# PengNi/deepsignal-plant

Hardware: NVIDIA B200
Metric: classified sites/sec (ModelBiLSTM both_bilstm bn13_sn16 hidden 256) (higher is better)
Workload: dtype f16 operands / f32 accumulate

## Files before the change

deepsignal_plant_b200/csrc/kernels_tc.cu:

```cuda
#include "tc.cuh"
#include "tc_prims.cuh"
#include <vector>
#include <cstring>
#include <cstdlib>

namespace dsp {

using namespace tc;

namespace {

constexpr int TILE = 128;
constexpr int SLAB_BYTES = TILE * SLAB_ROW_BYTES;
constexpr int HSLAB_BYTES = SLAB_BYTES / 2;
constexpr int EPI_WARPS = 16;
constexpr int NTHREADS = 128 + EPI_WARPS * 32;
constexpr int CPT = 128 / (EPI_WARPS / 4);
constexpr int UPT = CPT / 4;
constexpr float LOG2E = 1.4426950408889634f;
constexpr uint16_t PAIR_MASK = 3;

#ifndef DSP_POLY_MASK
#define DSP_POLY_MASK 0
#endif
#ifndef DSP_POLY_MASK_BRANCH
#define DSP_POLY_MASK_BRANCH 3
#endif
#ifndef DSP_POLY_MASK_L0
#define DSP_POLY_MASK_L0 DSP_POLY_MASK
#endif
#ifndef DSP_PW32_ALL
#define DSP_PW32_ALL 0
#endif
#ifndef DSP_DIR_INTERLEAVE
#define DSP_DIR_INTERLEAVE 1
#endif
#ifndef DSP_MERGE_RCP
#define DSP_MERGE_RCP 1
#endif
#ifndef DSP_TANH_APPROX
#define DSP_TANH_APPROX 2
#endif

struct LayerParams {
    const uint8_t* x_img;
    const uint8_t* w_img;
    const float* bias;
    const float* h0;
    const float* c0;
    uint64_t seed;
    uint32_t rng_call;
    uint32_t rng_slot;
    int64_t site_base;
    int64_t state_dir_stride;
    uint8_t* y_img;
    float* hfinal;
    int64_t n;
    int T;
    int xk16;
    int y_slabs;
    int y_col_off;
    int write_y;
    const float* w2t;
    const float* b2;
    float* logits;
    float* probs;
    int32_t* labels;
    int num_classes;
};

enum { MODE_LSTM = 0, MODE_FC = 1, MODE_HEAD = 2 };
constexpr int HEAD_MAX_CLASSES = 8;
template <int KSX, int MODE> struct RingCfg {
    static constexpr int STG = KSX >= 8 ? 2 : 4;
    static constexpr int NST = KSX >= 8 ? (MODE == 2 ? 4 : 5) : (MODE == 1 ? 2 : 4);
    static constexpr int XB = (MODE == 1 && KSX <= 4) ? 2 : 1;
};

__device__ __forceinline__ float4 philox_normal4(uint32_t c0, uint32_t c1, uint32_t c2, uint32_t c3, uint32_t k0, uint32_t k1) {
#pragma unroll
    for (int r = 0; r < 10; ++r) {
        const uint32_t hi0 = __umulhi(0xD2511F53u, c0), lo0 = 0xD2511F53u * c0;
        const uint32_t hi1 = __umulhi(0xCD9E8D57u, c2), lo1 = 0xCD9E8D57u * c2;
        c0 = hi1 ^ c1 ^ k0; c1 = lo1; c2 = hi0 ^ c3 ^ k1; c3 = lo0;
        k0 += 0x9E3779B9u; k1 += 0xBB67AE85u;
    }
    const float u0 = ((float)c0 + 1.0f) * 2.3283064365386963e-10f, u1 = (float)c1 * 2.3283064365386963e-10f;
    const float u2 = ((float)c2 + 1.0f) * 2.3283064365386963e-10f, u3 = (float)c3 * 2.3283064365386963e-10f;
    const float r0 = sqrtf(-2.0f * __logf(u0)), r1 = sqrtf(-2.0f * __logf(u2));
    float s0, cs0, s1, cs1;
    __sincosf(6.283185307179586f * u1, &s0, &cs0);
    __sincosf(6.283185307179586f * u3, &s1, &cs1);
    return make_float4(r0 * cs0, r0 * s0, r1 * cs1, r1 * s1);
}

template <bool POLY, bool HI_CLAMP>
__device__ __forceinline__ float2 exp2_pair(float2 x) {
    if constexpr (POLY) {
        x.x = fmaxf(fminf(x.x, 40.f), -126.f);
        x.y = fmaxf(fminf(x.y, 40.f), -126.f);
        const float MG = 12582912.f;
        const float2 t = add2(x, make_float2(MG, MG));
        const float2 r = add2(t, make_float2(-MG, -MG));
        const float2 f = fma2(r, make_float2(-1.f, -1.f), x);
        float2 q = fma2(make_float2(0.0013390863f, 0.0013390863f), f, make_float2(0.009676032f, 0.009676032f));
        q = fma2(q, f, make_float2(0.05550357f, 0.05550357f));
        q = fma2(q, f, make_float2(0.24022107f, 0.24022107f));
        q = fma2(q, f, make_float2(0.6931472f, 0.6931472f));
        q = fma2(q, f, make_float2(1.0000001f, 1.0000001f));
        q.x = __int_as_float(__float_as_int(q.x) + (__float_as_int(t.x) << 23));
        q.y = __int_as_float(__float_as_int(q.y) + (__float_as_int(t.y) << 23));
        return q;
    } else {
        if constexpr (HI_CLAMP) { x.x = fminf(x.x, 40.f); x.y = fminf(x.y, 40.f); }
        return make_float2(ex2_approx(x.x), ex2_approx(x.y));
    }
}

__device__ __forceinline__ float tanh_approx(float x) {
    float y;
    asm("tanh.approx.f32 %0, %1;" : "=f"(y) : "f"(x));
    return y;
}
__host__ __device__ inline float gate_scale(int g) {
#if DSP_TANH_APPROX == 2
    return g == 2 ? 1.f : 0.5f;
#elif DSP_TANH_APPROX == 1
    return g == 2 ? -2.f * 1.4426950408889634f : (g == 3 ? 0.5f : -1.4426950408889634f);
#else
    return g == 2 ? -2.f * 1.4426950408889634f : -1.4426950408889634f;
#endif
}

template <int PM>
__device__ __forceinline__ void lstm_cell2(float2 ai, float2 af, float2 ag, float2 ao, float2& c, float2& h) {
    const float2 ONE = make_float2(1.f, 1.f), NEG1 = make_float2(-1.f, -1.f);
#ifdef DSP_EPI_STUB
    c = fma2(af, make_float2(1e-3f, 1e-3f), c);
    h = fma2(add2(ai, add2(ag, ao)), make_float2(1e-2f, 1e-2f), mul2(c, make_float2(1e-3f, 1e-3f)));
    return;
#endif
#if DSP_TANH_APPROX == 2
    {
        const float2 HALF = make_float2(0.5f, 0.5f);
        const float2 si = fma2(make_float2(tanh_approx(ai.x), tanh_approx(ai.y)), HALF, HALF);
        const float2 sf = fma2(make_float2(tanh_approx(af.x), tanh_approx(af.y)), HALF, HALF);
        const float2 so = fma2(make_float2(tanh_approx(ao.x), tanh_approx(ao.y)), HALF, HALF);
        const float2 tg = make_float2(tanh_approx(ag.x), tanh_approx(ag.y));
        c = fma2(sf, c, mul2(si, tg));
        h = mul2(so, make_float2(tanh_approx(c.x), tanh_approx(c.y)));
        return;
    }
#endif
#if DSP_MERGE_RCP
    constexpr bool CLAMP_IF = true;
#else
    constexpr bool CLAMP_IF = false;
#endif
    const float2 ei = exp2_pair<((PM >> 2) & 1) != 0, CLAMP_IF>(ai);
    const float2 ef = exp2_pair<((PM >> 3) & 1) != 0, CLAMP_IF>(af);
    const float2 eg = exp2_pair<(PM & 1) != 0, true>(ag);
    const float2 eo = exp2_pair<((PM >> 4) & 1) != 0, false>(ao);
#if DSP_MERGE_RCP
    const float2 F = add2(ef, ONE);
    const float2 AG = mul2(add2(ei, ONE), add2(eg, ONE));
    const float2 num = fma2(c, AG, mul2(fma2(eg, NEG1, ONE), F));
    const float2 den = mul2(F, AG);
    const float2 cn = mul2(num, make_float2(rcp_approx(den.x), rcp_approx(den.y)));
#else
    const float2 F = add2(ef, ONE);
    const float2 sf = make_float2(rcp_approx(F.x), rcp_approx(F.y));
    const float2 AG = mul2(add2(ei, ONE), add2(eg, ONE));
    const float2 rg = make_float2(rcp_approx(AG.x), rcp_approx(AG.y));
    const float2 ig = mul2(fma2(eg, NEG1, ONE), rg);
    const float2 cn = fma2(sf, c, ig);
#endif
    c = cn;
#if DSP_TANH_APPROX == 1
    {
        const float2 HALF = make_float2(0.5f, 0.5f);
        const float2 so = fma2(make_float2(tanh_approx(ao.x), tanh_approx(ao.y)), HALF, HALF);
        h = mul2(so, make_float2(tanh_approx(cn.x), tanh_approx(cn.y)));
        return;
    }
#endif
    const float2 ec = exp2_pair<((PM >> 1) & 1) != 0, true>(mul2(cn, make_float2(-2.f * LOG2E, -2.f * LOG2E)));
    const float2 D = mul2(add2(eo, ONE), add2(ec, ONE));
    const float2 rd = make_float2(rcp_approx(D.x), rcp_approx(D.y));
    h = mul2(fma2(ec, NEG1, ONE), rd);
}

template <int KSX, int H, int MODE, int NOUT>
__global__ void __launch_bounds__(NTHREADS, 1)
layer_kernel(const LayerParams p) {
    constexpr bool IS_FC = MODE != MODE_LSTM;
    constexpr int STG = RingCfg<KSX, MODE>::STG, NST = RingCfg<KSX, MODE>::NST, XB = RingCfg<KSX, MODE>::XB;
    constexpr int NXS = KSX * XB;
    constexpr int NCH = IS_FC ? NOUT / 128 : H / 32;
    constexpr int KSH = IS_FC ? 0 : H / 64;
    constexpr int KS = KSX + KSH;
    constexpr int W_STEP = NCH * KS;
    constexpr int NBIAS = NCH * 128;
    constexpr uint32_t IDESC = make_idesc_f16(256, 128);
    static_assert(W_STEP % STG == 0, "a step must be a whole number of ring stages");
    static_assert(IS_FC || NCH % 2 == 0, "chunks are issued in pairs");
    static_assert(EPI_WARPS == 16 && CPT == 32 && UPT == 8, "the epilogue code below is written for 32-column slices");

    extern __shared__ __align__(1024) uint8_t smem_raw[];
    uint8_t* smem = (uint8_t*)(((uintptr_t)smem_raw + 1023) & ~(uintptr_t)1023);
    uint8_t* s_x = smem;
    uint8_t* s_w = smem + (size_t)NXS * SLAB_BYTES;
    float* s_bias = reinterpret_cast<float*>(s_w + (size_t)NST * STG * HSLAB_BYTES);
    __shared__ __align__(8) uint64_t bars[2 * NST + 2 * NXS + 5];
    __shared__ uint32_t tmem_base_s;
    const uint32_t b_wfull = smem_u32(&bars[0]), b_wempty = smem_u32(&bars[NST]);
    const uint32_t b_xfull = smem_u32(&bars[2 * NST]), b_xempty = smem_u32(&bars[2 * NST + NXS]);
    const uint32_t b_accfull = smem_u32(&bars[2 * NST + 2 * NXS]), b_accempty = b_accfull + 16;
    const uint32_t b_hready = b_accfull + 32;

    const int tid = threadIdx.x, warp = tid >> 5, lane = tid & 31;
#if DSP_DIR_INTERLEAVE
    const int dir = IS_FC ? 0 : (int)((blockIdx.x >> 1) & 1u);
    const int tile = IS_FC ? (int)blockIdx.x : (int)(((blockIdx.x >> 2) << 1) | (blockIdx.x & 1u));
#else
    const int tile = blockIdx.x, dir = IS_FC ? 0 : blockIdx.y;
#endif
    const int T = p.T;
    const uint32_t crank = cluster_ctarank();

    if (tid == 0) {
        const uint32_t both = crank == 0 ? 2u : 1u;
        for (int i = 0; i < NST; ++i) { mbar_init(b_wfull + 8 * i, both); mbar_init(b_wempty + 8 * i, 1); }
        for (int i = 0; i < NXS; ++i) { mbar_init(b_xfull + 8 * i, both); mbar_init(b_xempty + 8 * i, 1); }
        for (int i = 0; i < 2; ++i) { mbar_init(b_accfull + 8 * i, 1); mbar_init(b_accempty + 8 * i, 2 * EPI_WARPS); }
        mbar_init(b_hready, 2 * EPI_WARPS);
        mbar_fence_init();
    }
    if (warp == 3) tmem_alloc_pair(smem_u32(&tmem_base_s), 512);
    tc_fence_before();
    __syncthreads();
    cluster_sync_all();
    tc_fence_after();
    const uint32_t tmem = tmem_base_s;
    griddep_launch_dependents();
    const uint32_t t_acc = tmem;
    const uint32_t t_h = tmem + 256;

    if (warp < 4) {
        asm volatile("setmaxnreg.dec.sync.aligned.u32 32;");
        if (warp == 0) {
            if (elect_one()) {
                const size_t total = (size_t)(MODE == MODE_HEAD ? T : 1) * W_STEP;
                const uint8_t* wsrc = p.w_img + ((size_t)dir * 2 + crank) * total * HSLAB_BYTES;
                uint32_t stage = 0, phase = 0;
                for (int step = 0; step < T; ++step) {
                    const uint8_t* src = wsrc + (size_t)(MODE == MODE_HEAD ? step : 0) * W_STEP * HSLAB_BYTES;
                    for (int s = 0; s < W_STEP; s += STG) {
                        mbar_wait(b_wempty + 8 * stage, phase ^ 1);
                        mbar_arrive_expect_tx(b_wfull + 8 * stage, STG * HSLAB_BYTES);
                        bulk_g2s(smem_u32(s_w + (size_t)stage * STG * HSLAB_BYTES), src, STG * HSLAB_BYTES, b_wfull + 8 * stage);
                        src += (size_t)STG * HSLAB_BYTES;
                        if (++stage == NST) { stage = 0; phase ^= 1; }
                    }
                }
            }
        } else if (warp == 2) {
            if (elect_one()) {
                griddep_wait();
                for (int step = 0; step < T; ++step) {
                    const int t = dir ? (T - 1 - step) : step;
                    const uint8_t* xsrc = (MODE == MODE_HEAD)
                        ? p.x_img + ((size_t)tile * 2 + (step == 1 ? 1 : 0)) * KSX * SLAB_BYTES
                        : p.x_img + ((size_t)tile * T + t) * KSX * SLAB_BYTES;
                    const int xbuf = step % XB, xround = step / XB;
                    for (int j = 0; j < KSX; ++j) {
                        const int xi = xbuf * KSX + j;
                        mbar_wait(b_xempty + 8 * xi, (xround & 1) ^ 1);
                        mbar_arrive_expect_tx(b_xfull + 8 * xi, SLAB_BYTES);
                        bulk_g2s(smem_u32(s_x + (size_t)xi * SLAB_BYTES), xsrc + (size_t)j * SLAB_BYTES, SLAB_BYTES, b_xfull + 8 * xi);
                    }
                }
            }
        } else if (warp == 1 && crank != 0) {
            const uint32_t r_wfull = mapa_u32(b_wfull, 0), r_xfull = mapa_u32(b_xfull, 0);
            uint32_t stage = 0, phase = 0;
            for (int step = 0; step < T; ++step) {
                for (int j = 0; j < KSX; ++j) {
                    const int xi = (step % XB) * KSX + j;
                    mbar_wait(b_xfull + 8 * xi, (step / XB) & 1);
                    if (lane == 0) mbar_arrive_cluster(r_xfull + 8 * xi);
                }
                for (int s = 0; s < W_STEP; s += STG) {
                    mbar_wait(b_wfull + 8 * stage, phase);
                    if (lane == 0) mbar_arrive_cluster(r_wfull + 8 * stage);
                    if (++stage == NST) { stage = 0; phase ^= 1; }
                }
            }
        } else if (warp == 1) {
            const bool leader = elect_one();
            const uint32_t a_lo0 = smem_desc_lo(smem_u32(s_x)), b_lo0 = smem_desc_lo(smem_u32(s_w));
            const int xk16 = p.xk16;
            uint32_t stage = 0, phase = 0, in_stage = 0;
            auto w_acquire = [&]() -> uint32_t {
                if (in_stage == 0) { mbar_wait_cluster(b_wfull + 8 * stage, phase); tc_fence_after(); }
                return b_lo0 + (stage * STG + in_stage) * (uint32_t)(HSLAB_BYTES >> 4);
            };
            auto w_release = [&]() {
                if (++in_stage == STG) {
                    if (leader) mma2_commit(b_wempty + 8 * stage, PAIR_MASK);
                    in_stage = 0;
                    if (++stage == NST) { stage = 0; phase ^= 1; }
                }
                __syncwarp();
            };
            auto issue_x = [&](uint32_t acc, bool fresh, bool first_use, bool last_use, int step) {
#pragma unroll
                for (int j = 0; j < KSX; ++j) {
                    const int xi = (step % XB) * KSX + j;
                    if (first_use) { mbar_wait_cluster(b_xfull + 8 * xi, (step / XB) & 1); tc_fence_after(); }
                    const uint32_t bl = w_acquire();
                    if (leader) {
                        const uint32_t al = a_lo0 + (uint32_t)xi * (SLAB_BYTES >> 4);
                        const int nk = (KSX * 4 == xk16) ? 4 : min(4, xk16 - 4 * j);
#pragma unroll
                        for (int k = 0; k < 4; ++k) {
                            if (k < nk) {
                                if (j == 0 && k == 0 && fresh) mma2_ss_lo<0>(acc, al, bl, IDESC);
                                else mma2_ss_lo<1>(acc, al + k * 2, bl + k * 2, IDESC);
                            }
                        }
                        if (last_use) mma2_commit(b_xempty + 8 * xi, PAIR_MASK);
                    }
                    w_release();
                }
            };
            for (int step = 0; step < T; ++step) {
                if constexpr (MODE == MODE_LSTM) {
                    const uint32_t a_t = t_h + (uint32_t)(step & 1) * 128u;
                    for (int pr = 0; pr < NCH / 2; ++pr) {
                        const uint32_t use = (uint32_t)(step * (NCH / 2) + pr);
#pragma unroll
                        for (int e = 0; e < 2; ++e) {
                            mbar_wait_cluster(b_accempty + 8 * e, (use & 1u) ^ 1u);
                            tc_fence_after();
                            issue_x(t_acc + e * 128u, true, pr == 0 && e == 0, pr == NCH / 2 - 1 && e == 1, step);
                        }
                        if (pr == 0) { mbar_wait_cluster(b_hready, step & 1); tc_fence_after(); }
#pragma unroll
                        for (int e = 0; e < 2; ++e) {
#pragma unroll
                            for (int j = 0; j < KSH; ++j) {
                                const uint32_t bl = w_acquire();
                                if (leader) {
#pragma unroll
                                    for (int k = 0; k < 4; ++k)
                                        mma2_ts_lo<1>(t_acc + e * 128u, a_t + (uint32_t)(j * 32 + k * 8), bl + k * 2, IDESC);
                                }
                                w_release();
                            }
                            if (leader) mma2_commit(b_accfull + 8 * e, PAIR_MASK);
                            __syncwarp();
                        }
                    }
                } else {
                    for (int ch = 0; ch < NCH; ++ch) {
                        const uint32_t g = (MODE == MODE_HEAD) ? (uint32_t)ch : (uint32_t)(step * NCH + ch);
                        const uint32_t buf = g & 1u, use = g >> 1;
                        const bool fresh = (MODE != MODE_HEAD) || step == 0;
                        if (MODE != MODE_HEAD) { mbar_wait_cluster(b_accempty + 8 * buf, (use & 1u) ^ 1u); tc_fence_after(); }
                        issue_x(t_acc + buf * 128u, fresh, ch == 0, ch == NCH - 1, step);
                        if (leader && (MODE != MODE_HEAD || step == T - 1)) mma2_commit(b_accfull + 8 * buf, PAIR_MASK);
                        __syncwarp();
                    }
                }
            }
        }
    } else {
        asm volatile("setmaxnreg.inc.sync.aligned.u32 112;");
        const int ew = warp - 4;
        const int q = warp & 3;
        const int sl = ew >> 2;
        const int row = q * 32 + lane;
        const int64_t site = (int64_t)tile * TILE + row;
        const bool valid = site < p.n;
        const uint32_t lane_addr = (uint32_t)(q * 32) << 16;
        const uint32_t r_accempty = mapa_u32(b_accempty, 0), r_hready = mapa_u32(b_hready, 0);

        for (int i = tid - 128; i < NBIAS; i += EPI_WARPS * 32) s_bias[i] = p.bias[(size_t)dir * NBIAS + i];
        asm volatile("bar.sync 1, %0;" ::"n"(EPI_WARPS * 32) : "memory");

        if constexpr (MODE == MODE_HEAD) {
            __shared__ float head_part[EPI_WARPS / 4][TILE][HEAD_MAX_CLASSES];
            const int C = p.num_classes;
            float part_sum[HEAD_MAX_CLASSES];
#pragma unroll
            for (int cc = 0; cc < HEAD_MAX_CLASSES; ++cc) part_sum[cc] = 0.f;
#pragma unroll
            for (int ch = 0; ch < NCH; ++ch) {
                const uint32_t buf = (uint32_t)ch & 1u, use = (uint32_t)ch >> 1;
                mbar_wait(b_accfull + 8 * buf, use & 1u);
                tc_fence_after();
                uint32_t v[32];
                tmem_ld32(t_acc + buf * 128u + lane_addr + (uint32_t)(sl * CPT), v);
                tmem_ld_wait();
#pragma unroll
                for (int j = 0; j < 32; ++j) {
                    const int col = ch * 128 + sl * CPT + j;
                    const float z = fmaxf(__uint_as_float(v[j]) + s_bias[col], 0.f);
#pragma unroll
                    for (int cc = 0; cc < HEAD_MAX_CLASSES; ++cc)
                        if (cc < C) part_sum[cc] = fmaf(z, __ldg(p.w2t + (size_t)col * C + cc), part_sum[cc]);
                }
            }
#pragma unroll
            for (int cc = 0; cc < HEAD_MAX_CLASSES; ++cc) head_part[sl][row][cc] = part_sum[cc];
            asm volatile("bar.sync 1, %0;" ::"n"(EPI_WARPS * 32) : "memory");
            if (sl == 0 && valid) {
                float lg[HEAD_MAX_CLASSES];
                float mx = -3.0e38f;
                int arg = 0;
#pragma unroll
                for (int cc = 0; cc < HEAD_MAX_CLASSES; ++cc) {
                    lg[cc] = 0.f;
                    if (cc < C) {
                        float a = __ldg(p.b2 + cc);
#pragma unroll
                        for (int s4 = 0; s4 < EPI_WARPS / 4; ++s4) a += head_part[s4][row][cc];
                        lg[cc] = a;
                        if (lg[cc] > mx) { mx = lg[cc]; arg = cc; }
                    }
                }
                float sum = 0.f;
#pragma unroll
                for (int cc = 0; cc < HEAD_MAX_CLASSES; ++cc) if (cc < C) sum += expf(lg[cc] - mx);
#pragma unroll
                for (int cc = 0; cc < HEAD_MAX_CLASSES; ++cc)
                    if (cc < C) {
                        p.logits[site * C + cc] = lg[cc];
                        p.probs[site * C + cc] = expf(lg[cc] - mx) / sum;
                    }
                if (p.labels) p.labels[site] = arg;
            }
        } else if constexpr (MODE == MODE_FC) {
            for (int step = 0; step < T; ++step) {
                uint8_t* ybase = p.y_img + ((size_t)tile * T + step) * p.y_slabs * SLAB_BYTES;
#pragma unroll
                for (int ch = 0; ch < NCH; ++ch) {
                    const uint32_t g = (uint32_t)(step * NCH + ch);
                    const uint32_t buf = g & 1u, use = g >> 1;
                    mbar_wait(b_accfull + 8 * buf, use & 1u);
                    tc_fence_after();
                    const int col0 = p.y_col_off + ch * 128 + sl * CPT;
                    uint8_t* yslab = ybase + (size_t)(col0 >> 6) * SLAB_BYTES + row * SLAB_ROW_BYTES;
                    uint32_t v[32];
                    tmem_ld32(t_acc + buf * 128u + lane_addr + (uint32_t)(sl * CPT), v);
                    tmem_ld_wait();
                    tc_fence_before();
                    __syncwarp();
                    if (lane == 0) mbar_arrive_cluster(r_accempty + 8 * buf);
                    const float* bs = s_bias + ch * 128 + sl * CPT;
#pragma unroll
                    for (int c8 = 0; c8 < 4; ++c8) {
                        uint32_t o[4];
#pragma unroll
                        for (int e = 0; e < 4; ++e) {
                            const int j = c8 * 8 + e * 2;
                            const float a = fmaxf(__uint_as_float(v[j]) + bs[j], 0.f);
                            const float b = fmaxf(__uint_as_float(v[j + 1]) + bs[j + 1], 0.f);
                            o[e] = pack_half2(a, b);
                        }
                        const int chunk = ((col0 & 63) >> 3) + c8;
                        *reinterpret_cast<uint4*>(yslab + ((chunk ^ (row & 7)) << 4)) = make_uint4(o[0], o[1], o[2], o[3]);
                    }
                }
            }
        } else {
            float2 c2[NCH][UPT / 2];
            const bool draw = p.h0 == nullptr;
            const uint64_t gs = (uint64_t)(p.site_base + site);
            const uint32_t k0 = (uint32_t)p.seed, k1 = (uint32_t)(p.seed >> 32);
            const uint32_t slot0 = (p.rng_slot + (uint32_t)dir) << 16;
            if (draw) {
#pragma unroll 1
                for (int i = 0; i < NCH * (UPT / 4); ++i) {
                    const int unit = (i / (UPT / 4)) * 32 + sl * UPT + (i % (UPT / 4)) * 4;
                    const float4 hq = philox_normal4((uint32_t)gs, (uint32_t)(gs >> 32), slot0 | (uint32_t)(unit >> 2), p.rng_call, k0, k1);
                    tmem_st2(t_h + lane_addr + (uint32_t)(unit >> 1), pack_half2(hq.x, hq.y), pack_half2(hq.z, hq.w));
                }
                tmem_st_wait();
            } else {
                const float* h0 = p.h0 + (size_t)dir * p.state_dir_stride + (size_t)site * H;
                const float* c0 = p.c0 + (size_t)dir * p.state_dir_stride + (size_t)site * H;
#pragma unroll
                for (int ch = 0; ch < NCH; ++ch) {
                    const int u0 = ch * 32 + sl * UPT;
                    float4 cv0 = make_float4(0.f, 0.f, 0.f, 0.f), cv1 = cv0, hq0 = cv0, hq1 = cv0;
                    if (valid) {
                        cv0 = *reinterpret_cast<const float4*>(c0 + u0); cv1 = *reinterpret_cast<const float4*>(c0 + u0 + 4);
                        hq0 = *reinterpret_cast<const float4*>(h0 + u0); hq1 = *reinterpret_cast<const float4*>(h0 + u0 + 4);
                    }
                    c2[ch][0] = make_float2(cv0.x, cv0.y); c2[ch][1] = make_float2(cv0.z, cv0.w);
                    c2[ch][2] = make_float2(cv1.x, cv1.y); c2[ch][3] = make_float2(cv1.z, cv1.w);
                    tmem_st4(t_h + lane_addr + (uint32_t)(u0 >> 1), pack_half2(hq0.x, hq0.y), pack_half2(hq0.z, hq0.w),
                             pack_half2(hq1.x, hq1.y), pack_half2(hq1.z, hq1.w));
                }
                tmem_st_wait();
            }
            tc_fence_before();
            __syncwarp();
            if (lane == 0) mbar_arrive_cluster(r_hready);
            if (draw) {
                const uint32_t t_park = t_h + 128u + lane_addr;
#pragma unroll 1
                for (int i = 0; i < NCH * (UPT / 4); ++i) {
                    const int unit = (i / (UPT / 4)) * 32 + sl * UPT + (i % (UPT / 4)) * 4;
                    const float4 cv = philox_normal4((uint32_t)gs, (uint32_t)(gs >> 32), slot0 | (uint32_t)(unit >> 2) | 0x8000u, p.rng_call, k0, k1);
                    tmem_st2(t_park + (uint32_t)(unit >> 1), pack_half2(cv.x, cv.y), pack_half2(cv.z, cv.w));
                }
                tmem_st_wait();
#pragma unroll
                for (int ch = 0; ch < NCH; ++ch) {
                    uint32_t v[4];
                    tmem_ld4(t_park + (uint32_t)((ch * 32 + sl * UPT) >> 1), v);
                    tmem_ld_wait();
#pragma unroll
                    for (int j = 0; j < UPT / 2; ++j) {
                        const __half2 hh = *reinterpret_cast<const __half2*>(&v[j]);
                        c2[ch][j] = make_float2(__low2float(hh), __high2float(hh));
                    }
                }
            }
            const uint32_t s_bias_u32 = smem_u32(s_bias) + (uint32_t)(sl * CPT * 4);
            for (int step = 0; step < T; ++step) {
                const int t = dir ? (T - 1 - step) : step;
                const bool last = (step == T - 1);
                uint8_t* ybase = p.y_img + ((size_t)tile * (p.write_y == 2 ? 2 : T) + (p.write_y == 2 ? 0 : t)) * p.y_slabs * SLAB_BYTES
                                 + row * SLAB_ROW_BYTES;
                const bool do_write = p.write_y == 1 || (p.write_y == 2 && last);
                const uint32_t t_hnext = t_h + (uint32_t)((step + 1) & 1) * 128u + lane_addr;
#pragma unroll
                for (int ch = 0; ch < NCH; ++ch) {
                    const uint32_t buf = (uint32_t)ch & 1u;
                    const uint32_t use = (uint32_t)(step * (NCH / 2) + (ch >> 1));
                    mbar_wait(b_accfull + 8 * buf, use & 1u);
                    tc_fence_after();
                    const int u0 = ch * 32 + sl * UPT;
                    float2 h2[UPT / 2];
                    constexpr int PW = (H == 128 || DSP_PW32_ALL) ? 32 : 16;
#pragma unroll
                    for (int part = 0; part < CPT / PW; ++part) {
                        uint32_t v[PW];
                        if constexpr (PW == 32) tmem_ld32(t_acc + buf * 128u + lane_addr + (uint32_t)(sl * CPT), reinterpret_cast<uint32_t(&)[32]>(v));
                        else tmem_ld16(t_acc + buf * 128u + lane_addr + (uint32_t)(sl * CPT + part * 16), reinterpret_cast<uint32_t(&)[16]>(v));
                        float4 bq[PW / 4];
#pragma unroll
                        for (int i = 0; i < PW / 4; ++i) bq[i] = lds128(s_bias_u32 + (uint32_t)((ch * 128 + part * PW + i * 4) * 4));
                        tmem_ld_wait();
                        if (part == CPT / PW - 1) {
                            tc_fence_before();
                            __syncwarp();
                            if (lane == 0) mbar_arrive_cluster(r_accempty + 8 * buf);
                        }
#pragma unroll
                        for (int qq = 0; qq < PW / 8; ++qq) {
                            const float4 b0 = bq[2 * qq], b1 = bq[2 * qq + 1];
                            const float2 ai = add2(make_float2(__uint_as_float(v[qq * 8 + 0]), __uint_as_float(v[qq * 8 + 1])), make_float2(b0.x, b0.y));
                            const float2 af = add2(make_float2(__uint_as_float(v[qq * 8 + 2]), __uint_as_float(v[qq * 8 + 3])), make_float2(b0.z, b0.w));
                            const float2 ag = add2(make_float2(__uint_as_float(v[qq * 8 + 4]), __uint_as_float(v[qq * 8 + 5])), make_float2(b1.x, b1.y));
                            const float2 ao = add2(make_float2(__uint_as_float(v[qq * 8 + 6]), __uint_as_float(v[qq * 8 + 7])), make_float2(b1.z, b1.w));
                            lstm_cell2<(H == 128) ? DSP_POLY_MASK_BRANCH : (KSX == 4 ? DSP_POLY_MASK_L0 : DSP_POLY_MASK)>(ai, af, ag, ao, c2[ch][part * (PW / 8) + qq], h2[part * (PW / 8) + qq]);
                        }
                    }
                    uint32_t pk[UPT / 2];
#pragma unroll
                    for (int j = 0; j < UPT / 2; ++j) pk[j] = pack_half2(h2[j].x, h2[j].y);
                    tmem_st4(t_hnext + (uint32_t)(u0 >> 1), pk[0], pk[1], pk[2], pk[3]);
                    if (do_write) {
                        const int col = dir * H + u0;
                        uint8_t* yslab = ybase + (size_t)(col >> 6) * SLAB_BYTES;
                        const int chunk = (col & 63) >> 3;
                        *reinterpret_cast<uint4*>(yslab + (((chunk) ^ (row & 7)) << 4)) = make_uint4(pk[0], pk[1], pk[2], pk[3]);
                        if (p.write_y == 2) {
                            uint32_t lo[UPT / 2];
#pragma unroll
                            for (int j = 0; j < UPT / 2; ++j) {
                                const __half2 hh = *reinterpret_cast<const __half2*>(&pk[j]);
                                lo[j] = pack_half2(h2[j].x - __low2float(hh), h2[j].y - __high2float(hh));
                            }
                            uint8_t* lslab = yslab + (size_t)p.y_slabs * SLAB_BYTES;
                            *reinterpret_cast<uint4*>(lslab + (((chunk) ^ (row & 7)) << 4)) = make_uint4(lo[0], lo[1], lo[2], lo[3]);
                        }
                    }
                    if (last && p.hfinal != nullptr && valid) {
                        float* hf = p.hfinal + (size_t)site * (2 * H) + dir * H + u0;
#pragma unroll
                        for (int j = 0; j < UPT / 2; j += 2)
                            *reinterpret_cast<float4*>(hf + 2 * j) = make_float4(h2[j].x, h2[j].y, h2[j + 1].x, h2[j + 1].y);
                    }
                }
                tmem_st_wait();
                tc_fence_before();
                __syncwarp();
                if (lane == 0) mbar_arrive_cluster(r_hready);
            }
        }
    }
    tc_fence_before();
    __syncthreads();
    cluster_sync_all();
    if (warp == 3) tmem_dealloc_pair(tmem, 512);
}

constexpr int BR_H = 128, BR_NW = 64, BR_NCH = BR_H / 16, BR_KSH = BR_H / 64;
constexpr int QSLAB_BYTES = 32 * SLAB_ROW_BYTES;
constexpr int BR_STG = 4, BR_NST = 6;

template <int KSX>
__global__ void __launch_bounds__(NTHREADS, 1)
branch_kernel(const LayerParams p) {
    constexpr int KS = KSX + BR_KSH;
    constexpr int PAIR_UNITS = 4 * KSX + 4 * BR_KSH;
    constexpr int W_STEP = (BR_NCH / 2) * PAIR_UNITS;
    constexpr int NBIAS = 2 * BR_NCH * BR_NW;
    constexpr uint32_t IDESC = make_idesc_f16(256, BR_NW);
    static_assert(W_STEP % BR_STG == 0 && KS * 2 == PAIR_UNITS / 2, "stream layout");

    extern __shared__ __align__(1024) uint8_t smem_raw[];
    uint8_t* smem = (uint8_t*)(((uintptr_t)smem_raw + 1023) & ~(uintptr_t)1023);
    uint8_t* s_x = smem;
    uint8_t* s_w = smem + (size_t)2 * KSX * SLAB_BYTES;
    float* s_bias = reinterpret_cast<float*>(s_w + (size_t)BR_NST * BR_STG * QSLAB_BYTES);
    __shared__ __align__(8) uint64_t bars[2 * BR_NST + 4 * KSX + 10];
    __shared__ uint32_t tmem_base_s;
    const uint32_t b_wfull = smem_u32(&bars[0]), b_wempty = smem_u32(&bars[BR_NST]);
    const uint32_t b_xfull = smem_u32(&bars[2 * BR_NST]), b_xempty = b_xfull + 8 * 2 * KSX;
    const uint32_t b_accfull = b_xempty + 8 * 2 * KSX, b_accempty = b_accfull + 32;
    const uint32_t b_hready = b_accempty + 32;

    const int tid = threadIdx.x, warp = tid >> 5, lane = tid & 31;
    const int tile = blockIdx.x;
    const int T = p.T;
    const uint32_t crank = cluster_ctarank();

    if (tid == 0) {
        const uint32_t both = crank == 0 ? 2u : 1u;
        for (int i = 0; i < BR_NST; ++i) { mbar_init(b_wfull + 8 * i, both); mbar_init(b_wempty + 8 * i, 1); }
        for (int i = 0; i < 2 * KSX; ++i) { mbar_init(b_xfull + 8 * i, both); mbar_init(b_xempty + 8 * i, 1); }
        for (int i = 0; i < 4; ++i) { mbar_init(b_accfull + 8 * i, 1); mbar_init(b_accempty + 8 * i, EPI_WARPS); }
        for (int i = 0; i < 2; ++i) mbar_init(b_hready + 8 * i, EPI_WARPS);
        mbar_fence_init();
    }
    if (warp == 3) tmem_alloc_pair(smem_u32(&tmem_base_s), 512);
    tc_fence_before();
    __syncthreads();
    cluster_sync_all();
    tc_fence_after();
    const uint32_t tmem = tmem_base_s;
    griddep_launch_dependents();
    auto t_acc = [&](int d, int e) -> uint32_t { return tmem + (uint32_t)(d * 128 + e * 64); };
    auto t_h = [&](int d, int b) -> uint32_t { return tmem + 256u + (uint32_t)(d * 128 + b * 64); };

    if (warp < 4) {
        asm volatile("setmaxnreg.dec.sync.aligned.u32 32;");
        if (warp == 0) {
            if (elect_one()) {
                const uint8_t* wsrc = p.w_img + (size_t)crank * W_STEP * QSLAB_BYTES;
                uint32_t stage = 0, phase = 0;
                for (int step = 0; step < T; ++step) {
                    const uint8_t* src = wsrc;
                    for (int s = 0; s < W_STEP; s += BR_STG) {
                        mbar_wait(b_wempty + 8 * stage, phase ^ 1);
                        mbar_arrive_expect_tx(b_wfull + 8 * stage, BR_STG * QSLAB_BYTES);
                        bulk_g2s(smem_u32(s_w + (size_t)stage * BR_STG * QSLAB_BYTES), src, BR_STG * QSLAB_BYTES, b_wfull + 8 * stage);
                        src += (size_t)BR_STG * QSLAB_BYTES;
                        if (++stage == BR_NST) { stage = 0; phase ^= 1; }
                    }
                }
            }
        } else if (warp == 2) {
            if (elect_one()) {
                griddep_wait();
                for (int step = 0; step < T; ++step)
                    for (int d = 0; d < 2; ++d) {
                        const int t = d ? (T - 1 - step) : step;
                        const uint8_t* xsrc = p.x_img + ((size_t)tile * T + t) * KSX * SLAB_BYTES;
                        for (int j = 0; j < KSX; ++j) {
                            const uint32_t o = 8u * (uint32_t)(d * KSX + j);
                            mbar_wait(b_xempty + o, (step & 1) ^ 1);
                            mbar_arrive_expect_tx(b_xfull + o, SLAB_BYTES);
                            bulk_g2s(smem_u32(s_x + (size_t)(d * KSX + j) * SLAB_BYTES), xsrc + (size_t)j * SLAB_BYTES, SLAB_BYTES, b_xfull + o);
                        }
                    }
            }
        } else if (warp == 1 && crank != 0) {
            const uint32_t r_wfull = mapa_u32(b_wfull, 0), r_xfull = mapa_u32(b_xfull, 0);
            uint32_t stage = 0, phase = 0;
            for (int step = 0; step < T; ++step) {
                for (int i = 0; i < 2 * KSX; ++i) {
                    mbar_wait(b_xfull + 8 * i, step & 1);
                    if (lane == 0) mbar_arrive_cluster(r_xfull + 8 * i);
                }
                for (int s = 0; s < W_STEP; s += BR_STG) {
                    mbar_wait(b_wfull + 8 * stage, phase);
                    if (lane == 0) mbar_arrive_cluster(r_wfull + 8 * stage);
                    if (++stage == BR_NST) { stage = 0; phase ^= 1; }
                }
            }
        } else if (warp == 1) {
            const bool leader = elect_one();
            const uint32_t a_lo0 = smem_desc_lo(smem_u32(s_x)), b_lo0 = smem_desc_lo(smem_u32(s_w));
            const int xk16 = p.xk16;
            uint32_t stage = 0, phase = 0, in_stage = 0;
            auto w_acquire = [&]() -> uint32_t {
                if (in_stage == 0) { mbar_wait_cluster(b_wfull + 8 * stage, phase); tc_fence_after(); }
                return b_lo0 + (stage * BR_STG + in_stage) * (uint32_t)(QSLAB_BYTES >> 4);
            };
            auto w_release = [&]() {
                if (++in_stage == BR_STG) {
                    if (leader) mma2_commit(b_wempty + 8 * stage, PAIR_MASK);
                    in_stage = 0;
                    if (++stage == BR_NST) { stage = 0; phase ^= 1; }
                }
                __syncwarp();
            };
            for (int step = 0; step < T; ++step) {
                for (int pr = 0; pr < BR_NCH / 2; ++pr) {
                    const uint32_t use = (uint32_t)(step * (BR_NCH / 2) + pr);
#pragma unroll
                    for (int d = 0; d < 2; ++d)
#pragma unroll
                        for (int e = 0; e < 2; ++e) {
                            mbar_wait_cluster(b_accempty + 8 * (d * 2 + e), (use & 1u) ^ 1u);
                            tc_fence_after();
#pragma unroll
                            for (int j = 0; j < KSX; ++j) {
                                const uint32_t xo = 8u * (uint32_t)(d * KSX + j);
                                if (pr == 0 && e == 0) { mbar_wait_cluster(b_xfull + xo, step & 1); tc_fence_after(); }
                                const uint32_t bl = w_acquire();
                                if (leader) {
                                    const uint32_t al = a_lo0 + (uint32_t)(d * KSX + j) * (SLAB_BYTES >> 4);
                                    const int nk = (KSX * 4 == xk16) ? 4 : min(4, xk16 - 4 * j);
#pragma unroll
                                    for (int k = 0; k < 4; ++k) {
                                        if (k < nk) {
                                            if (j == 0 && k == 0) mma2_ss_lo<0>(t_acc(d, e), al, bl, IDESC);
                                            else mma2_ss_lo<1>(t_acc(d, e), al + k * 2, bl + k * 2, IDESC);
                                        }
                                    }
                                    if (pr == BR_NCH / 2 - 1 && e == 1) mma2_commit(b_xempty + xo, PAIR_MASK);
                                }
                                w_release();
                            }
                        }
#pragma unroll
                    for (int d = 0; d < 2; ++d) {
                        if (pr == 0) { mbar_wait_cluster(b_hready + 8 * d, step & 1); tc_fence_after(); }
                        const uint32_t a_t = t_h(d, step & 1);
#pragma unroll
                        for (int e = 0; e < 2; ++e) {
#pragma unroll
                            for (int j = 0; j < BR_KSH; ++j) {
                                const uint32_t bl = w_acquire();
                                if (leader) {
#pragma unroll
                                    for (int k = 0; k < 4; ++k)
                                        mma2_ts_lo<1>(t_acc(d, e), a_t + (uint32_t)(j * 32 + k * 8), bl + k * 2, IDESC);
                                }
                                w_release();
                            }
                            if (leader) mma2_commit(b_accfull + 8 * (d * 2 + e), PAIR_MASK);
                            __syncwarp();
                        }
                    }
                }
            }
        }
    } else {
        asm volatile("setmaxnreg.inc.sync.aligned.u32 112;");
        const int ew = warp - 4;
        const int d = ew >> 3;
        const int q = warp & 3;
        const int half = (ew >> 2) & 1;
        const int row = q * 32 + lane;
        const int64_t site = (int64_t)tile * TILE + row;
        const bool valid = site < p.n;
        const uint32_t lane_addr = (uint32_t)(q * 32) << 16;
        const uint32_t r_accempty = mapa_u32(b_accempty, 0) + 16u * (uint32_t)d, r_hready = mapa_u32(b_hready, 0) + 8u * (uint32_t)d;
        const uint32_t b_myfull = b_accfull + 16u * (uint32_t)d;

        for (int i = tid - 128; i < NBIAS; i += EPI_WARPS * 32) s_bias[i] = p.bias[i];
        asm volatile("bar.sync 1, %0;" ::"n"(EPI_WARPS * 32) : "memory");

        constexpr int UPT = 8;
        float2 c2[BR_NCH][UPT / 2];
        const bool draw = p.h0 == nullptr;
        const uint64_t gs = (uint64_t)(p.site_base + site);
        const uint32_t k0 = (uint32_t)p.seed, k1 = (uint32_t)(p.seed >> 32);
        const uint32_t slot0 = (p.rng_slot + (uint32_t)d) << 16;
        if (draw) {
#pragma unroll 1
            for (int i = 0; i < BR_NCH * (UPT / 4); ++i) {
                const int unit = (i >> 1) * 16 + half * UPT + (i & 1) * 4;
                const float4 hq = philox_normal4((uint32_t)gs, (uint32_t)(gs >> 32), slot0 | (uint32_t)(unit >> 2), p.rng_call, k0, k1);
                tmem_st2(t_h(d, 0) + lane_addr + (uint32_t)(unit >> 1), pack_half2(hq.x, hq.y), pack_half2(hq.z, hq.w));
            }
            tmem_st_wait();
        } else {
            const float* h0 = p.h0 + (size_t)d * p.state_dir_stride + (size_t)site * BR_H;
            const float* c0 = p.c0 + (size_t)d * p.state_dir_stride + (size_t)site * BR_H;
#pragma unroll
            for (int ch = 0; ch < BR_NCH; ++ch) {
                const int u0 = ch * 16 + half * UPT;
                float4 cv0 = make_float4(0.f, 0.f, 0.f, 0.f), cv1 = cv0, hq0 = cv0, hq1 = cv0;
                if (valid) {
                    cv0 = *reinterpret_cast<const float4*>(c0 + u0); cv1 = *reinterpret_cast<const float4*>(c0 + u0 + 4);
                    hq0 = *reinterpret_cast<const float4*>(h0 + u0); hq1 = *reinterpret_cast<const float4*>(h0 + u0 + 4);
                }
                c2[ch][0] = make_float2(cv0.x, cv0.y); c2[ch][1] = make_float2(cv0.z, cv0.w);
                c2[ch][2] = make_float2(cv1.x, cv1.y); c2[ch][3] = make_float2(cv1.z, cv1.w);
                tmem_st4(t_h(d, 0) + lane_addr + (uint32_t)(u0 >> 1), pack_half2(hq0.x, hq0.y), pack_half2(hq0.z, hq0.w),
                         pack_half2(hq1.x, hq1.y), pack_half2(hq1.z, hq1.w));
            }
            tmem_st_wait();
        }
        tc_fence_before();
        __syncwarp();
        if (lane == 0) mbar_arrive_cluster(r_hready);
        if (draw) {
            const uint32_t t_park = t_h(d, 1) + lane_addr;
#pragma unroll 1
            for (int i = 0; i < BR_NCH * (UPT / 4); ++i) {
                const int unit = (i >> 1) * 16 + half * UPT + (i & 1) * 4;
                const float4 cv = philox_normal4((uint32_t)gs, (uint32_t)(gs >> 32), slot0 | (uint32_t)(unit >> 2) | 0x8000u, p.rng_call, k0, k1);
                tmem_st2(t_park + (uint32_t)(unit >> 1), pack_half2(cv.x, cv.y), pack_half2(cv.z, cv.w));
            }
            tmem_st_wait();
#pragma unroll
            for (int ch = 0; ch < BR_NCH; ++ch) {
                uint32_t v[4];
                tmem_ld4(t_park + (uint32_t)((ch * 16 + half * UPT) >> 1), v);
                tmem_ld_wait();
#pragma unroll
                for (int j = 0; j < UPT / 2; ++j) {
                    const __half2 hh = *reinterpret_cast<const __half2*>(&v[j]);
                    c2[ch][j] = make_float2(__low2float(hh), __high2float(hh));
                }
            }
        }
        const uint32_t s_bias_u32 = smem_u32(s_bias) + (uint32_t)((d * BR_NCH * BR_NW + half * 32) * 4);
        for (int step = 0; step < T; ++step) {
            const int t = d ? (T - 1 - step) : step;
            uint8_t* ybase = p.y_img + ((size_t)tile * T + t) * p.y_slabs * SLAB_BYTES + row * SLAB_ROW_BYTES;
            const uint32_t t_hnext = t_h(d, (step + 1) & 1) + lane_addr;
#pragma unroll
            for (int ch = 0; ch < BR_NCH; ++ch) {
                const int e = ch & 1;
                const uint32_t use = (uint32_t)(step * (BR_NCH / 2) + (ch >> 1));
                mbar_wait(b_myfull + 8 * e, use & 1u);
                tc_fence_after();
                const int u0 = ch * 16 + half * UPT;
                float2 h2[UPT / 2];
#pragma unroll
                for (int part = 0; part < 2; ++part) {
                    uint32_t v[16];
                    tmem_ld16(t_acc(d, e) + lane_addr + (uint32_t)(half * 32 + part * 16), v);
                    float4 bq[4];
#pragma unroll
                    for (int i = 0; i < 4; ++i) bq[i] = lds128(s_bias_u32 + (uint32_t)((ch * BR_NW + part * 16 + i * 4) * 4));
                    tmem_ld_wait();
                    if (part == 1) {
                        tc_fence_before();
                        __syncwarp();
                        if (lane == 0) mbar_arrive_cluster(r_accempty + 8 * e);
                    }
#pragma unroll
                    for (int qq = 0; qq < 2; ++qq) {
                        const float4 b0 = bq[2 * qq], b1 = bq[2 * qq + 1];
                        const float2 ai = add2(make_float2(__uint_as_float(v[qq * 8 + 0]), __uint_as_float(v[qq * 8 + 1])), make_float2(b0.x, b0.y));
                        const float2 af = add2(make_float2(__uint_as_float(v[qq * 8 + 2]), __uint_as_float(v[qq * 8 + 3])), make_float2(b0.z, b0.w));
                        const float2 ag = add2(make_float2(__uint_as_float(v[qq * 8 + 4]), __uint_as_float(v[qq * 8 + 5])), make_float2(b1.x, b1.y));
                        const float2 ao = add2(make_float2(__uint_as_float(v[qq * 8 + 6]), __uint_as_float(v[qq * 8 + 7])), make_float2(b1.z, b1.w));
                        lstm_cell2<DSP_POLY_MASK_BRANCH>(ai, af, ag, ao, c2[ch][part * 2 + qq], h2[part * 2 + qq]);
                    }
                }
                uint32_t pk[UPT / 2];
#pragma unroll
                for (int j = 0; j < UPT / 2; ++j) pk[j] = pack_half2(h2[j].x, h2[j].y);
                tmem_st4(t_hnext + (uint32_t)(u0 >> 1), pk[0], pk[1], pk[2], pk[3]);
                const int col = d * BR_H + u0;
                uint8_t* yslab = ybase + (size_t)(col >> 6) * SLAB_BYTES;
                *reinterpret_cast<uint4*>(yslab + ((((col & 63) >> 3) ^ (row & 7)) << 4)) = make_uint4(pk[0], pk[1], pk[2], pk[3]);
            }
            tmem_st_wait();
            tc_fence_before();
            __syncwarp();
            if (lane == 0) mbar_arrive_cluster(r_hready);
        }
    }
    tc_fence_before();
    __syncthreads();
    cluster_sync_all();
    if (warp == 3) tmem_dealloc_pair(tmem, 512);
}

struct FusedBranchParams {
    const uint8_t* x_img[2];
    const uint8_t* w_img[2];
    const float* bias[2];
    const float* h0[2];
    const float* c0[2];
    int64_t state_dir_stride[2];
    uint32_t rng_slot[2];
    int xk16[2];
    uint8_t* y_img[2];
    const uint8_t* fcw_img[2];
    const float* fcb[2];
    uint8_t* comb_img;
    uint64_t seed;
    uint32_t rng_call;
    int64_t site_base;
    int64_t n;
    int T;
};

__global__ void __launch_bounds__(NTHREADS, 1)
branch_fused_kernel(const FusedBranchParams p) {
    constexpr int KSX = 1;
    constexpr int KS = KSX + BR_KSH;
    constexpr int PAIR_UNITS = 4 * KSX + 4 * BR_KSH;
    constexpr int W_STEP = (BR_NCH / 2) * PAIR_UNITS;
    constexpr int NBIAS = 2 * BR_NCH * BR_NW;
    constexpr uint32_t IDESC = make_idesc_f16(256, BR_NW);
    constexpr uint32_t IDESC_FC = make_idesc_f16(256, 128);
    constexpr int FC_KS = 4;
    static_assert(W_STEP % BR_STG == 0 && KS * 2 == PAIR_UNITS / 2, "stream layout");
    static_assert(2 * KSX * SLAB_BYTES + BR_NST * BR_STG * QSLAB_BYTES == 2 * FC_KS * SLAB_BYTES, "tail A buffers alias x + ring exactly");

    extern __shared__ __align__(1024) uint8_t smem_raw[];
    uint8_t* smem = (uint8_t*)(((uintptr_t)smem_raw + 1023) & ~(uintptr_t)1023);
    uint8_t* s_x = smem;
    uint8_t* s_w = smem + (size_t)2 * KSX * SLAB_BYTES;
    uint8_t* s_a = smem;
    uint8_t* s_wfc = smem + (size_t)2 * FC_KS * SLAB_BYTES;
    float* s_bias = reinterpret_cast<float*>(s_wfc + (size_t)FC_KS * HSLAB_BYTES);
    float* s_fcb = s_bias + NBIAS;
    __shared__ __align__(8) uint64_t bars[2 * BR_NST + 4 * KSX + 10 + 10];
    __shared__ uint32_t tmem_base_s;
    const uint32_t b_wfull = smem_u32(&bars[0]), b_wempty = smem_u32(&bars[BR_NST]);
    const uint32_t b_xfull = smem_u32(&bars[2 * BR_NST]), b_xempty = b_xfull + 8 * 2 * KSX;
    const uint32_t b_accfull = b_xempty + 8 * 2 * KSX, b_accempty = b_accfull + 32;
    const uint32_t b_hready = b_accempty + 32;
    const uint32_t b_tail = b_hready + 16;
    const uint32_t b_wfc = b_tail + 8;
    const uint32_t b_afull = b_wfc + 8, b_aempty = b_afull + 16;
    const uint32_t b_faccfull = b_aempty + 16, b_faccempty = b_faccfull + 16;

    const int tid = threadIdx.x, warp = tid >> 5, lane = tid & 31;
    const int br = (int)((blockIdx.x >> 1) & 1u);
    const int tile = (int)(((blockIdx.x >> 2) << 1) | (blockIdx.x & 1u));
    const int T = p.T;
    const uint32_t crank = cluster_ctarank();

    if (tid == 0) {
        const uint32_t both = crank == 0 ? 2u : 1u;
        for (int i = 0; i < BR_NST; ++i) { mbar_init(b_wfull + 8 * i, both); mbar_init(b_wempty + 8 * i, 1); }
        for (int i = 0; i < 2 * KSX; ++i) { mbar_init(b_xfull + 8 * i, both); mbar_init(b_xempty + 8 * i, 1); }
        for (int i = 0; i < 4; ++i) { mbar_init(b_accfull + 8 * i, 1); mbar_init(b_accempty + 8 * i, EPI_WARPS); }
        for (int i = 0; i < 2; ++i) mbar_init(b_hready + 8 * i, EPI_WARPS);
        mbar_init(b_tail, EPI_WARPS);
        mbar_init(b_wfc, both);
        for (int i = 0; i < 2; ++i) {
            mbar_init(b_afull + 8 * i, both); mbar_init(b_aempty + 8 * i, 1);
            mbar_init(b_faccfull + 8 * i, 1); mbar_init(b_faccempty + 8 * i, 2 * EPI_WARPS);
        }
        mbar_fence_init();
    }
    if (warp == 3) tmem_alloc_pair(smem_u32(&tmem_base_s), 512);
    tc_fence_before();
    __syncthreads();
    cluster_sync_all();
    tc_fence_after();
    const uint32_t tmem = tmem_base_s;
    griddep_launch_dependents();
    auto t_acc = [&](int d, int e) -> uint32_t { return tmem + (uint32_t)(d * 128 + e * 64); };
    auto t_h = [&](int d, int b) -> uint32_t { return tmem + 256u + (uint32_t)(d * 128 + b * 64); };
    const uint8_t* x_img = p.x_img[br];
    uint8_t* y_img = p.y_img[br];

    if (warp < 4) {
        asm volatile("setmaxnreg.dec.sync.aligned.u32 32;");
        if (warp == 0) {
            if (elect_one()) {
                mbar_arrive_expect_tx(b_wfc, FC_KS * HSLAB_BYTES);
                bulk_g2s(smem_u32(s_wfc), p.fcw_img[br] + (size_t)crank * FC_KS * HSLAB_BYTES, FC_KS * HSLAB_BYTES, b_wfc);
                const uint8_t* wsrc = p.w_img[br] + (size_t)crank * W_STEP * QSLAB_BYTES;
                uint32_t stage = 0, phase = 0;
                for (int step = 0; step < T; ++step) {
                    const uint8_t* src = wsrc;
                    for (int s = 0; s < W_STEP; s += BR_STG) {
                        mbar_wait(b_wempty + 8 * stage, phase ^ 1);
                        mbar_arrive_expect_tx(b_wfull + 8 * stage, BR_STG * QSLAB_BYTES);
                        bulk_g2s(smem_u32(s_w + (size_t)stage * BR_STG * QSLAB_BYTES), src, BR_STG * QSLAB_BYTES, b_wfull + 8 * stage);
                        src += (size_t)BR_STG * QSLAB_BYTES;
                        if (++stage == BR_NST) { stage = 0; phase ^= 1; }
                    }
                }
            }
        } else if (warp == 2) {
            if (elect_one()) {
                griddep_wait();
                for (int step = 0; step < T; ++step)
                    for (int d = 0; d < 2; ++d) {
                        const int t = d ? (T - 1 - step) : step;
                        const uint8_t* xsrc = x_img + ((size_t)tile * T + t) * KSX * SLAB_BYTES;
                        for (int j = 0; j < KSX; ++j) {
                            const uint32_t o = 8u * (uint32_t)(d * KSX + j);
                            mbar_wait(b_xempty + o, (step & 1) ^ 1);
                            mbar_arrive_expect_tx(b_xfull + o, SLAB_BYTES);
                            bulk_g2s(smem_u32(s_x + (size_t)(d * KSX + j) * SLAB_BYTES), xsrc + (size_t)j * SLAB_BYTES, SLAB_BYTES, b_xfull + o);
                        }
                    }
                mbar_wait(b_tail, 0);
                for (int t = 0; t < T; ++t) {
                    const uint32_t buf = (uint32_t)t & 1u;
                    mbar_wait(b_aempty + 8 * buf, ((uint32_t)(t >> 1) & 1u) ^ 1u);
                    mbar_arrive_expect_tx(b_afull + 8 * buf, FC_KS * SLAB_BYTES);
                    bulk_g2s(smem_u32(s_a + (size_t)buf * FC_KS * SLAB_BYTES), y_img + ((size_t)tile * T + t) * FC_KS * SLAB_BYTES,
                             FC_KS * SLAB_BYTES, b_afull + 8 * buf);
                }
            }
        } else if (warp == 1 && crank != 0) {
            const uint32_t r_wfull = mapa_u32(b_wfull, 0), r_xfull = mapa_u32(b_xfull, 0);
            uint32_t stage = 0, phase = 0;
            for (int step = 0; step < T; ++step) {
                for (int i = 0; i < 2 * KSX; ++i) {
                    mbar_wait(b_xfull + 8 * i, step & 1);
                    if (lane == 0) mbar_arrive_cluster(r_xfull + 8 * i);
                }
                for (int s = 0; s < W_STEP; s += BR_STG) {
                    mbar_wait(b_wfull + 8 * stage, phase);
                    if (lane == 0) mbar_arrive_cluster(r_wfull + 8 * stage);
                    if (++stage == BR_NST) { stage = 0; phase ^= 1; }
                }
            }
            const uint32_t r_wfc = mapa_u32(b_wfc, 0), r_afull = mapa_u32(b_afull, 0);
            mbar_wait(b_wfc, 0);
            if (lane == 0) mbar_arrive_cluster(r_wfc);
            for (int t = 0; t < T; ++t) {
                const uint32_t buf = (uint32_t)t & 1u;
                mbar_wait(b_afull + 8 * buf, (uint32_t)(t >> 1) & 1u);
                if (lane == 0) mbar_arrive_cluster(r_afull + 8 * buf);
            }
        } else if (warp == 1) {
            const bool leader = elect_one();
            const uint32_t a_lo0 = smem_desc_lo(smem_u32(s_x)), b_lo0 = smem_desc_lo(smem_u32(s_w));
            const int xk16 = p.xk16[br];
            uint32_t stage = 0, phase = 0, in_stage = 0;
            auto w_acquire = [&]() -> uint32_t {
                if (in_stage == 0) { mbar_wait_cluster(b_wfull + 8 * stage, phase); tc_fence_after(); }
                return b_lo0 + (stage * BR_STG + in_stage) * (uint32_t)(QSLAB_BYTES >> 4);
            };
            auto w_release = [&]() {
                if (++in_stage == BR_STG) {
                    if (leader) mma2_commit(b_wempty + 8 * stage, PAIR_MASK);
                    in_stage = 0;
                    if (++stage == BR_NST) { stage = 0; phase ^= 1; }
                }
                __syncwarp();
            };
            for (int step = 0; step < T; ++step) {
                for (int pr = 0; pr < BR_NCH / 2; ++pr) {
                    const uint32_t use = (uint32_t)(step * (BR_NCH / 2) + pr);
#pragma unroll
                    for (int d = 0; d < 2; ++d)
#pragma unroll
                        for (int e = 0; e < 2; ++e) {
                            mbar_wait_cluster(b_accempty + 8 * (d * 2 + e), (use & 1u) ^ 1u);
                            tc_fence_after();
#pragma unroll
                            for (int j = 0; j < KSX; ++j) {
                                const uint32_t xo = 8u * (uint32_t)(d * KSX + j);
                                if (pr == 0 && e == 0) { mbar_wait_cluster(b_xfull + xo, step & 1); tc_fence_after(); }
                                const uint32_t bl = w_acquire();
                                if (leader) {
                                    const uint32_t al = a_lo0 + (uint32_t)(d * KSX + j) * (SLAB_BYTES >> 4);
                                    const int nk = (KSX * 4 == xk16) ? 4 : min(4, xk16 - 4 * j);
#pragma unroll
                                    for (int k = 0; k < 4; ++k) {
                                        if (k < nk) {
                                            if (j == 0 && k == 0) mma2_ss_lo<0>(t_acc(d, e), al, bl, IDESC);
                                            else mma2_ss_lo<1>(t_acc(d, e), al + k * 2, bl + k * 2, IDESC);
                                        }
                                    }
                                    if (pr == BR_NCH / 2 - 1 && e == 1) mma2_commit(b_xempty + xo, PAIR_MASK);
                                }
                                w_release();
                            }
                        }
#pragma unroll
                    for (int d = 0; d < 2; ++d) {
                        if (pr == 0) { mbar_wait_cluster(b_hready + 8 * d, step & 1); tc_fence_after(); }
                        const uint32_t a_t = t_h(d, step & 1);
#pragma unroll
                        for (int e = 0; e < 2; ++e) {
#pragma unroll
                            for (int j = 0; j < BR_KSH; ++j) {
                                const uint32_t bl = w_acquire();
                                if (leader) {
#pragma unroll
                                    for (int k = 0; k < 4; ++k)
                                        mma2_ts_lo<1>(t_acc(d, e), a_t + (uint32_t)(j * 32 + k * 8), bl + k * 2, IDESC);
                                }
                                w_release();
                            }
                            if (leader) mma2_commit(b_accfull + 8 * (d * 2 + e), PAIR_MASK);
                            __syncwarp();
                        }
                    }
                }
            }
            const uint32_t fa_lo0 = smem_desc_lo(smem_u32(s_a)), fb_lo0 = smem_desc_lo(smem_u32(s_wfc));
            mbar_wait_cluster(b_wfc, 0);
            tc_fence_after();
            for (int t = 0; t < T; ++t) {
                const uint32_t buf = (uint32_t)t & 1u, use = (uint32_t)(t >> 1);
                mbar_wait_cluster(b_faccempty + 8 * buf, (use & 1u) ^ 1u);
                mbar_wait_cluster(b_afull + 8 * buf, use & 1u);
                tc_fence_after();
                if (leader) {
#pragma unroll
                    for (int j = 0; j < FC_KS; ++j) {
                        const uint32_t al = fa_lo0 + (buf * FC_KS + (uint32_t)j) * (SLAB_BYTES >> 4);
                        const uint32_t bl = fb_lo0 + (uint32_t)j * (HSLAB_BYTES >> 4);
#pragma unroll
                        for (int k = 0; k < 4; ++k) {
                            if (j == 0 && k == 0) mma2_ss_lo<0>(tmem + buf * 128u, al, bl, IDESC_FC);
                            else mma2_ss_lo<1>(tmem + buf * 128u, al + k * 2, bl + k * 2, IDESC_FC);
                        }
                    }
                    mma2_commit(b_aempty + 8 * buf, PAIR_MASK);
                    mma2_commit(b_faccfull + 8 * buf, PAIR_MASK);
                }
                __syncwarp();
            }
        }
    } else {
        asm volatile("setmaxnreg.inc.sync.aligned.u32 112;");
        const int ew = warp - 4;
        const int d = ew >> 3;
        const int q = warp & 3;
        const int half = (ew >> 2) & 1;
        const int row = q * 32 + lane;
        const int64_t site = (int64_t)tile * TILE + row;
        const bool valid = site < p.n;
        const uint32_t lane_addr = (uint32_t)(q * 32) << 16;
        const uint32_t r_accempty = mapa_u32(b_accempty, 0) + 16u * (uint32_t)d, r_hready = mapa_u32(b_hready, 0) + 8u * (uint32_t)d;
        const uint32_t b_myfull = b_accfull + 16u * (uint32_t)d;

        for (int i = tid - 128; i < NBIAS; i += EPI_WARPS * 32) s_bias[i] = p.bias[br][i];
        for (int i = tid - 128; i < 128; i += EPI_WARPS * 32) s_fcb[i] = p.fcb[br][i];
        asm volatile("bar.sync 1, %0;" ::"n"(EPI_WARPS * 32) : "memory");

        constexpr int UPT = 8;
        float2 c2[BR_NCH][UPT / 2];
        const bool draw = p.h0[br] == nullptr;
        const uint64_t gs = (uint64_t)(p.site_base + site);
        const uint32_t k0 = (uint32_t)p.seed, k1 = (uint32_t)(p.seed >> 32);
        const uint32_t slot0 = (p.rng_slot[br] + (uint32_t)d) << 16;
        if (draw) {
#pragma unroll 1
            for (int i = 0; i < BR_NCH * (UPT / 4); ++i) {
                const int unit = (i >> 1) * 16 + half * UPT + (i & 1) * 4;
                const float4 hq = philox_normal4((uint32_t)gs, (uint32_t)(gs >> 32), slot0 | (uint32_t)(unit >> 2), p.rng_call, k0, k1);
                tmem_st2(t_h(d, 0) + lane_addr + (uint32_t)(unit >> 1), pack_half2(hq.x, hq.y), pack_half2(hq.z, hq.w));
            }
            tmem_st_wait();
        } else {
            const float* h0 = p.h0[br] + (size_t)d * p.state_dir_stride[br] + (size_t)site * BR_H;
            const float* c0 = p.c0[br] + (size_t)d * p.state_dir_stride[br] + (size_t)site * BR_H;
#pragma unroll
            for (int ch = 0; ch < BR_NCH; ++ch) {
                const int u0 = ch * 16 + half * UPT;
                float4 cv0 = make_float4(0.f, 0.f, 0.f, 0.f), cv1 = cv0, hq0 = cv0, hq1 = cv0;
                if (valid) {
                    cv0 = *reinterpret_cast<const float4*>(c0 + u0); cv1 = *reinterpret_cast<const float4*>(c0 + u0 + 4);
                    hq0 = *reinterpret_cast<const float4*>(h0 + u0); hq1 = *reinterpret_cast<const float4*>(h0 + u0 + 4);
                }
                c2[ch][0] = make_float2(cv0.x, cv0.y); c2[ch][1] = make_float2(cv0.z, cv0.w);
                c2[ch][2] = make_float2(cv1.x, cv1.y); c2[ch][3] = make_float2(cv1.z, cv1.w);
                tmem_st4(t_h(d, 0) + lane_addr + (uint32_t)(u0 >> 1), pack_half2(hq0.x, hq0.y), pack_half2(hq0.z, hq0.w),
                         pack_half2(hq1.x, hq1.y), pack_half2(hq1.z, hq1.w));
            }
            tmem_st_wait();
        }
        tc_fence_before();
        __syncwarp();
        if (lane == 0) mbar_arrive_cluster(r_hready);
        if (draw) {
            const uint32_t t_park = t_h(d, 1) + lane_addr;
#pragma unroll 1
            for (int i = 0; i < BR_NCH * (UPT / 4); ++i) {
                const int unit = (i >> 1) * 16 + half * UPT + (i & 1) * 4;
                const float4 cv = philox_normal4((uint32_t)gs, (uint32_t)(gs >> 32), slot0 | (uint32_t)(unit >> 2) | 0x8000u, p.rng_call, k0, k1);
                tmem_st2(t_park + (uint32_t)(unit >> 1), pack_half2(cv.x, cv.y), pack_half2(cv.z, cv.w));
            }
            tmem_st_wait();
#pragma unroll
            for (int ch = 0; ch < BR_NCH; ++ch) {
                uint32_t v[4];
                tmem_ld4(t_park + (uint32_t)((ch * 16 + half * UPT) >> 1), v);
                tmem_ld_wait();
#pragma unroll
                for (int j = 0; j < UPT / 2; ++j) {
                    const __half2 hh = *reinterpret_cast<const __half2*>(&v[j]);
                    c2[ch][j] = make_float2(__low2float(hh), __high2float(hh));
                }
            }
        }
        const uint32_t s_bias_u32 = smem_u32(s_bias) + (uint32_t)((d * BR_NCH * BR_NW + half * 32) * 4);
        for (int step = 0; step < T; ++step) {
            const int t = d ? (T - 1 - step) : step;
            uint8_t* ybase = y_img + ((size_t)tile * T + t) * FC_KS * SLAB_BYTES + row * SLAB_ROW_BYTES;
            const uint32_t t_hnext = t_h(d, (step + 1) & 1) + lane_addr;
#pragma unroll
            for (int ch = 0; ch < BR_NCH; ++ch) {
                const int e = ch & 1;
                const uint32_t use = (uint32_t)(step * (BR_NCH / 2) + (ch >> 1));
                mbar_wait(b_myfull + 8 * e, use & 1u);
                tc_fence_after();
                const int u0 = ch * 16 + half * UPT;
                float2 h2[UPT / 2];
#pragma unroll
                for (int part = 0; part < 2; ++part) {
                    uint32_t v[16];
                    tmem_ld16(t_acc(d, e) + lane_addr + (uint32_t)(half * 32 + part * 16), v);
                    float4 bq[4];
#pragma unroll
                    for (int i = 0; i < 4; ++i) bq[i] = lds128(s_bias_u32 + (uint32_t)((ch * BR_NW + part * 16 + i * 4) * 4));
                    tmem_ld_wait();
                    if (part == 1) {
                        tc_fence_before();
                        __syncwarp();
                        if (lane == 0) mbar_arrive_cluster(r_accempty + 8 * e);
                    }
#pragma unroll
                    for (int qq = 0; qq < 2; ++qq) {
                        const float4 b0 = bq[2 * qq], b1 = bq[2 * qq + 1];
                        const float2 ai = add2(make_float2(__uint_as_float(v[qq * 8 + 0]), __uint_as_float(v[qq * 8 + 1])), make_float2(b0.x, b0.y));
                        const float2 af = add2(make_float2(__uint_as_float(v[qq * 8 + 2]), __uint_as_float(v[qq * 8 + 3])), make_float2(b0.z, b0.w));
                        const float2 ag = add2(make_float2(__uint_as_float(v[qq * 8 + 4]), __uint_as_float(v[qq * 8 + 5])), make_float2(b1.x, b1.y));
                        const float2 ao = add2(make_float2(__uint_as_float(v[qq * 8 + 6]), __uint_as_float(v[qq * 8 + 7])), make_float2(b1.z, b1.w));
                        lstm_cell2<DSP_POLY_MASK_BRANCH>(ai, af, ag, ao, c2[ch][part * 2 + qq], h2[part * 2 + qq]);
                    }
                }
                uint32_t pk[UPT / 2];
#pragma unroll
                for (int j = 0; j < UPT / 2; ++j) pk[j] = pack_half2(h2[j].x, h2[j].y);
                tmem_st4(t_hnext + (uint32_t)(u0 >> 1), pk[0], pk[1], pk[2], pk[3]);
                const int col = d * BR_H + u0;
                uint8_t* yslab = ybase + (size_t)(col >> 6) * SLAB_BYTES;
                *reinterpret_cast<uint4*>(yslab + ((((col & 63) >> 3) ^ (row & 7)) << 4)) = make_uint4(pk[0], pk[1], pk[2], pk[3]);
            }
            tmem_st_wait();
            tc_fence_before();
            __syncwarp();
            if (lane == 0) mbar_arrive_cluster(r_hready);
        }
        asm volatile("fence.proxy.async.global;" ::: "memory");
        __syncwarp();
        if (lane == 0) mbar_arrive(b_tail);
        {
            const int sl = ew >> 2;
            const uint32_t r_faccempty = mapa_u32(b_faccempty, 0);
            const int col0 = br * 128 + sl * 32;
            const float* bs = s_fcb + sl * 32;
            for (int t = 0; t < T; ++t) {
                const uint32_t buf = (uint32_t)t & 1u, use = (uint32_t)(t >> 1);
                mbar_wait(b_faccfull + 8 * buf, use & 1u);
                tc_fence_after();
                uint32_t v[32];
                tmem_ld32(tmem + buf * 128u + lane_addr + (uint32_t)(sl * 32), v);
                tmem_ld_wait();
                tc_fence_before();
                __syncwarp();
                if (lane == 0) mbar_arrive_cluster(r_faccempty + 8 * buf);
                uint8_t* yslab = p.comb_img + (((size_t)tile * T + t) * FC_KS + (size_t)(col0 >> 6)) * SLAB_BYTES + row * SLAB_ROW_BYTES;
#pragma unroll
                for (int c8 = 0; c8 < 4; ++c8) {
                    uint32_t o[4];
#pragma unroll
                    for (int e = 0; e < 4; ++e) {
                        const int j = c8 * 8 + e * 2;
                        const float a = fmaxf(__uint_as_float(v[j]) + bs[j], 0.f);
                        const float b = fmaxf(__uint_as_float(v[j + 1]) + bs[j + 1], 0.f);
                        o[e] = pack_half2(a, b);
                    }
                    const int chunk = ((col0 & 63) >> 3) + c8;
                    *reinterpret_cast<uint4*>(yslab + ((chunk ^ (row & 7)) << 4)) = make_uint4(o[0], o[1], o[2], o[3]);
                }
            }
        }
    }
    tc_fence_before();
    __syncthreads();
    cluster_sync_all();
    if (warp == 3) tmem_dealloc_pair(tmem, 512);
}

constexpr float SEQ_LEN_SCALE = 1.f / 32.f;
__device__ __forceinline__ float clamp_half(float v) { return fminf(fmaxf(v, -65504.f), 65504.f); }
__device__ __forceinline__ float half_residual(float v) { return v - __half2float(__float2half_rn(v)); }

__global__ void prep_images_kernel(const float* __restrict__ kmer, const float* __restrict__ means,
                                   const float* __restrict__ stds, const float* __restrict__ lens,
                                   const float* __restrict__ signals, const float* __restrict__ embed,
                                   int E, int vocab, int use_len, int split, int S, int T, int64_t n, int64_t n_pad,
                                   uint8_t* __restrict__ xseq_img, uint8_t* __restrict__ xsig_img) {
    const int64_t idx = (int64_t)blockIdx.x * blockDim.x + threadIdx.x;
    if (idx >= n_pad * T) return;
    const int64_t site = idx / T;
    const int t = (int)(idx - site * T);
    const int64_t tile = site >> 7;
    const int row = (int)(site & 127);
    const bool valid = site < n;
    const size_t slab = ((size_t)tile * T + t) * SLAB_BYTES;
    if (xseq_img) {
        float f[16];
#pragma unroll
        for (int i = 0; i < 16; ++i) f[i] = 0.f;
        if (valid) {
            int c = 0;
            if (E > 0) {
                long long code = (long long)kmer[site * T + t];
                code = code < 0 ? 0 : (code >= vocab ? vocab - 1 : code);
                for (int e = 0; e < E && c < 16; ++e) f[c++] = embed[code * E + e];
            }
            const int nsc = use_len ? 3 : 2;
            float sc[3];
            sc[0] = clamp_half(means[site * T + t]);
            sc[1] = clamp_half(stds[site * T + t]);
            sc[2] = use_len ? clamp_half(lens[site * T + t] * (split ? SEQ_LEN_SCALE : 1.f)) : 0.f;
            for (int i = 0; i < nsc && c + i < 16; ++i) {
                f[c + i] = sc[i];
                if (split) f[c + nsc + i] = half_residual(sc[i]);
            }
        }
        uint8_t* dst = xseq_img + slab + row * SLAB_ROW_BYTES;
#pragma unroll
        for (int chunk = 0; chunk < 2; ++chunk) {
            uint4 o;
            o.x = pack_half2(f[chunk * 8 + 0], f[chunk * 8 + 1]); o.y = pack_half2(f[chunk * 8 + 2], f[chunk * 8 + 3]);
            o.z = pack_half2(f[chunk * 8 + 4], f[chunk * 8 + 5]); o.w = pack_half2(f[chunk * 8 + 6], f[chunk * 8 + 7]);
            *reinterpret_cast<uint4*>(dst + ((chunk ^ (row & 7)) << 4)) = o;
        }
    }
    if (xsig_img) {
        const float* src = signals + (site * T + t) * S;
        uint8_t* dst = xsig_img + slab + row * SLAB_ROW_BYTES;
        const int nchunk = ((S + 15) / 16) * 2;
        const bool vec = (S & 3) == 0;
        for (int chunk = 0; chunk < nchunk; ++chunk) {
            float f[8];
            if (vec) {
#pragma unroll
                for (int h4 = 0; h4 < 2; ++h4) {
                    const int k = chunk * 8 + h4 * 4;
                    float4 v = make_float4(0.f, 0.f, 0.f, 0.f);
                    if (valid && k < S) v = __ldg(reinterpret_cast<const float4*>(src + k));
                    f[h4 * 4] = v.x; f[h4 * 4 + 1] = v.y; f[h4 * 4 + 2] = v.z; f[h4 * 4 + 3] = v.w;
                }
            } else {
#pragma unroll
                for (int i = 0; i < 8; ++i) { const int k = chunk * 8 + i; f[i] = (valid && k < S) ? src[k] : 0.f; }
            }
#pragma unroll
            for (int i = 0; i < 8; ++i) f[i] = clamp_half(f[i]);
            uint4 o;
            o.x = pack_half2(f[0], f[1]); o.y = pack_half2(f[2], f[3]); o.z = pack_half2(f[4], f[5]); o.w = pack_half2(f[6], f[7]);
            *reinterpret_cast<uint4*>(dst + ((chunk ^ (row & 7)) << 4)) = o;
        }
    }
}

struct TcLstmPack {
    uint8_t* w_img = nullptr;
    float* bias = nullptr;
    int KSX = 0, xk16 = 0;
    uint8_t* w_img_dual = nullptr;
    float* bias_dual = nullptr;
};
struct TcDensePack {
    uint8_t* w_img = nullptr;
    float* bias = nullptr;
    int KS = 0;
};
struct TcState {
    uint8_t* xseq_img = nullptr;
    uint8_t* xsig_img = nullptr;
    uint8_t* ybuf[2] = {nullptr, nullptr};
    uint8_t* comb_img = nullptr;
    float* hfinal = nullptr;
    uint8_t* hfin_img = nullptr;
    TcDensePack* head_pack = nullptr;
    bool tc_head = false;
    bool seq_split = false;
    bool pdl = true;
    int force_dual = -1;
    int64_t tiles = 0;
    std::vector<TcLstmPack*> lstm_packs;
    std::vector<TcDensePack*> dense_packs;
};

void put_half(std::vector<uint8_t>& img, size_t rank_base, size_t s, int n, int k, float v) {
    __half h = __float2half_rn(v);
    memcpy(&img[(rank_base + s) * HSLAB_BYTES + slab_offset_bytes((uint32_t)(n & 63), (uint32_t)k)], &h, 2);
}

int tc_alloc(Model* m, void** p, size_t bytes) {
    cudaError_t e = cudaMalloc(p, bytes ? bytes : 16);
    if (e != cudaSuccess) { set_error("cudaMalloc(%zu bytes) failed: %s", bytes, cudaGetErrorString(e)); return DSP_ERR_NOMEM; }
    m->device_allocs.push_back(*p);
    return DSP_OK;
}

template <int KSX, int H, int MODE, int NOUT>
int launch_layer(Model* m, const LayerParams& p, int64_t tiles, cudaStream_t st) {
    constexpr int NCH = MODE != MODE_LSTM ? NOUT / 128 : H / 32;
    const size_t smem = (size_t)KSX * RingCfg<KSX, MODE>::XB * SLAB_BYTES + (size_t)RingCfg<KSX, MODE>::NST * RingCfg<KSX, MODE>::STG * HSLAB_BYTES
                        + (size_t)NCH * 128 * sizeof(float) + 1024;
    auto kern = layer_kernel<KSX, H, MODE, NOUT>;
    DSP_CUDA(cudaFuncSetAttribute(kern, cudaFuncAttributeMaxDynamicSharedMemorySize, (int)smem));
    cudaLaunchConfig_t cfg{};
    const unsigned tiles2 = (unsigned)((tiles + 1) / 2 * 2);
#if DSP_DIR_INTERLEAVE
    cfg.gridDim = dim3(MODE != MODE_LSTM ? tiles2 : 2 * tiles2, 1);
#else
    cfg.gridDim = dim3(tiles2, MODE != MODE_LSTM ? 1 : 2);
#endif
    cfg.blockDim = dim3(NTHREADS);
    cfg.dynamicSmemBytes = smem;
    cfg.stream = st;
    cudaLaunchAttribute attr[2];
    attr[0].id = cudaLaunchAttributeClusterDimension;
    attr[0].val.clusterDim.x = 2; attr[0].val.clusterDim.y = 1; attr[0].val.clusterDim.z = 1;
    attr[1].id = cudaLaunchAttributeProgrammaticStreamSerialization;
    attr[1].val.programmaticStreamSerializationAllowed = 1;
    cfg.attrs = attr;
    cfg.numAttrs = ((TcState*)m->tc_state)->pdl ? 2 : 1;
    DSP_CUDA(cudaLaunchKernelEx(&cfg, kern, p));
    m->launches++;
    return DSP_OK;
}

template <int KSX>
int launch_branch(Model* m, const LayerParams& p, int64_t tiles, cudaStream_t st) {
    const size_t smem = (size_t)2 * KSX * SLAB_BYTES + (size_t)BR_NST * BR_STG * QSLAB_BYTES + (size_t)2 * BR_NCH * BR_NW * sizeof(float) + 1024;
    auto kern = branch_kernel<KSX>;
    DSP_CUDA(cudaFuncSetAttribute(kern, cudaFuncAttributeMaxDynamicSharedMemorySize, (int)smem));
    cudaLaunchConfig_t cfg{};
    cfg.gridDim = dim3((unsigned)((tiles + 1) / 2 * 2), 1);
    cfg.blockDim = dim3(NTHREADS);
    cfg.dynamicSmemBytes = smem;
    cfg.stream = st;
    cudaLaunchAttribute attr[2];
    attr[0].id = cudaLaunchAttributeClusterDimension;
    attr[0].val.clusterDim.x = 2; attr[0].val.clusterDim.y = 1; attr[0].val.clusterDim.z = 1;
    attr[1].id = cudaLaunchAttributeProgrammaticStreamSerialization;
    attr[1].val.programmaticStreamSerializationAllowed = 1;
    cfg.attrs = attr;
    cfg.numAttrs = ((TcState*)m->tc_state)->pdl ? 2 : 1;
    DSP_CUDA(cudaLaunchKernelEx(&cfg, kern, p));
    m->launches++;
    return DSP_OK;
}

int launch_branch_fused(Model* m, const FusedBranchParams& p, int64_t tiles, cudaStream_t st) {
    const size_t smem = (size_t)2 * 4 * SLAB_BYTES + (size_t)4 * HSLAB_BYTES + (size_t)(2 * BR_NCH * BR_NW + 128) * sizeof(float) + 1024;
    auto kern = branch_fused_kernel;
    DSP_CUDA(cudaFuncSetAttribute(kern, cudaFuncAttributeMaxDynamicSharedMemorySize, (int)smem));
    cudaLaunchConfig_t cfg{};
    cfg.gridDim = dim3((unsigned)(2 * ((tiles + 1) / 2 * 2)), 1);
    cfg.blockDim = dim3(NTHREADS);
    cfg.dynamicSmemBytes = smem;
    cfg.stream = st;
    cudaLaunchAttribute attr[2];
    attr[0].id = cudaLaunchAttributeClusterDimension;
    attr[0].val.clusterDim.x = 2; attr[0].val.clusterDim.y = 1; attr[0].val.clusterDim.z = 1;
    attr[1].id = cudaLaunchAttributeProgrammaticStreamSerialization;
    attr[1].val.programmaticStreamSerializationAllowed = 1;
    cfg.attrs = attr;
    cfg.numAttrs = ((TcState*)m->tc_state)->pdl ? 2 : 1;
    DSP_CUDA(cudaLaunchKernelEx(&cfg, kern, p));
    m->launches++;
    return DSP_OK;
}

int launch_lstm(Model* m, int KSX, int H, const LayerParams& p, int64_t tiles, cudaStream_t st) {
    if (H == 128) {
        if (KSX == 1) return launch_layer<1, 128, MODE_LSTM, 0>(m, p, tiles, st);
        if (KSX == 4) return launch_layer<4, 128, MODE_LSTM, 0>(m, p, tiles, st);
    } else if (H == 256) {
        if (KSX == 1) return launch_layer<1, 256, MODE_LSTM, 0>(m, p, tiles, st);
        if (KSX == 4) return launch_layer<4, 256, MODE_LSTM, 0>(m, p, tiles, st);
        if (KSX == 8) return launch_layer<8, 256, MODE_LSTM, 0>(m, p, tiles, st);
    }
    set_error("tcgen05 path: unsupported LSTM layer shape (x slabs %d, hidden %d)", KSX, H);
    return DSP_ERR_INVALID;
}

int launch_fc(Model* m, int KS, int NOUT, const LayerParams& p, int64_t tiles, cudaStream_t st) {
    if (KS == 4 && NOUT == 128) return launch_layer<4, 0, MODE_FC, 128>(m, p, tiles, st);
    if (KS == 8 && NOUT == 256) return launch_layer<8, 0, MODE_FC, 256>(m, p, tiles, st);
    set_error("tcgen05 path: unsupported dense shape (K slabs %d, N %d)", KS, NOUT);
    return DSP_ERR_INVALID;
}

}

int tc_create(Model* m) {
    const dsp_config& c = m->cfg;
    DSP_REQUIRE(c.hidden_size == 256, DSP_ERR_INVALID,
                "DSP_PRECISION_FP16 (tcgen05) supports hidden_size 256 (got %d); use DSP_PRECISION_FP32", c.hidden_size);
    DSP_REQUIRE(c.signal_len <= 64 && m->kseq <= 16, DSP_ERR_INVALID,
                "DSP_PRECISION_FP16 supports signal_len <= 64 and <= 16 sequence features per base");
    TcState* s = new TcState();
    m->tc_state = s;
    if (const char* e = getenv("DSP_B200_PDL")) s->pdl = atoi(e) != 0;
    if (const char* e = getenv("DSP_B200_BRANCH_DUAL")) s->force_dual = atoi(e) != 0;
    {
        const int e = c.is_base ? c.embedding_size : 0, nsc = c.is_signallen ? 3 : 2;
        s->seq_split = c.module != DSP_SIGNAL_BILSTM && e + 2 * nsc <= 16;
    }
    s->tiles = ((m->cap + TILE - 1) / TILE + 1) / 2 * 2;
    const size_t per_tile_t = (size_t)s->tiles * c.seq_len * SLAB_BYTES;
    int rc;
    if (c.module != DSP_SIGNAL_BILSTM) if ((rc = tc_alloc(m, (void**)&s->xseq_img, per_tile_t))) return rc;
    if (c.module != DSP_SEQ_BILSTM) if ((rc = tc_alloc(m, (void**)&s->xsig_img, per_tile_t))) return rc;
    if ((rc = tc_alloc(m, (void**)&s->ybuf[0], per_tile_t * 8))) return rc;
    if ((rc = tc_alloc(m, (void**)&s->ybuf[1], per_tile_t * 8))) return rc;
    if ((rc = tc_alloc(m, (void**)&s->comb_img, per_tile_t * 4))) return rc;
    if ((rc = tc_alloc(m, (void**)&s->hfinal, sizeof(float) * (size_t)s->tiles * TILE * 2 * c.hidden_size))) return rc;
    if ((rc = tc_alloc(m, (void**)&s->hfin_img, (size_t)s->tiles * 2 * (2 * c.hidden_size / 64) * SLAB_BYTES))) return rc;
    DSP_CUDA(cudaMemset(s->ybuf[0], 0, per_tile_t * 8));
    DSP_CUDA(cudaMemset(s->ybuf[1], 0, per_tile_t * 8));
    DSP_CUDA(cudaMemset(s->comb_img, 0, per_tile_t * 4));
    DSP_CUDA(cudaMemset(s->hfin_img, 0, (size_t)s->tiles * 2 * (2 * c.hidden_size / 64) * SLAB_BYTES));
    s->tc_head = c.num_classes <= HEAD_MAX_CLASSES;
    return DSP_OK;
}

bool tc_seq_split(const Model* m) {
    const TcState* s = (const TcState*)m->tc_state;
    return s && s->seq_split;
}

void tc_destroy(Model* m) {
    TcState* s = (TcState*)m->tc_state;
    if (!s) return;
    for (auto* p : s->lstm_packs) delete p;
    for (auto* p : s->dense_packs) delete p;
    delete s;
    m->tc_state = nullptr;
}

void tc_drop_packs(Model* m) {
    TcState* s = (TcState*)m->tc_state;
    if (!s) return;
    for (auto* p : s->lstm_packs) delete p;
    for (auto* p : s->dense_packs) delete p;
    s->lstm_packs.clear();
    s->dense_packs.clear();
    s->head_pack = nullptr;
}

int tc_pack_lstm_layer(Model* m, LstmLayer& L,
                       const float* wih0, const float* whh0, const float* bih0, const float* bhh0,
                       const float* wih1, const float* whh1, const float* bih1, const float* bhh1,
                       int split_first, int split_n, int len_col) {
    TcState* s = (TcState*)m->tc_state;
    const int H = L.H;
    int K = L.K;
    DSP_REQUIRE(H == 128 || H == 256, DSP_ERR_INVALID, "tcgen05 path: LSTM hidden size %d unsupported", H);
    std::vector<float> wext[2];
    if (split_n > 0) {
        const int K2 = K + split_n;
        const float* src[2] = {wih0, wih1};
        for (int d = 0; d < 2; ++d) {
            wext[d].assign((size_t)4 * H * K2, 0.f);
            for (int r = 0; r < 4 * H; ++r)
                for (int k = 0; k < K2; ++k) {
                    const int k0 = k < K ? k : split_first + (k - K);
                    wext[d][(size_t)r * K2 + k] = src[d][(size_t)r * K + k0] * (k0 == len_col ? 1.f / SEQ_LEN_SCALE : 1.f);
                }
        }
        wih0 = wext[0].data(); wih1 = wext[1].data();
        K = K2;
    }
    const int KSX = (K + 63) / 64, KSH = H / 64, KS = KSX + KSH, NCH = H / 32;
    DSP_REQUIRE(KSX == 1 || KSX == 4 || KSX == 8, DSP_ERR_INVALID, "tcgen05 path: LSTM input width %d unsupported", K);
    TcLstmPack* pk = new TcLstmPack();
    s->lstm_packs.push_back(pk);
    pk->KSX = KSX;
    pk->xk16 = (K + 15) / 16;
    const float* wih[2] = {wih0, wih1}; const float* whh[2] = {whh0, whh1};
    const float* bih[2] = {bih0, bih1}; const float* bhh[2] = {bhh0, bhh1};
    if (H == BR_H && KSX == 1) {
        const int pair_units = 4 * KSX + 4 * KSH;
        const size_t per_rank = (size_t)(BR_NCH / 2) * pair_units;
        std::vector<uint8_t> img((size_t)2 * per_rank * QSLAB_BYTES, 0);
        std::vector<float> bias((size_t)2 * BR_NCH * BR_NW);
        auto put = [&](int rank, size_t unit, int row, int k, float v) {
            __half h = __float2half_rn(v);
            memcpy(&img[((size_t)rank * per_rank + unit) * QSLAB_BYTES + slab_offset_bytes((uint32_t)row, (uint32_t)k)], &h, 2);
        };
        for (int d = 0; d < 2; ++d)
            for (int ch = 0; ch < BR_NCH; ++ch) {
                const size_t pair_base = (size_t)(ch >> 1) * pair_units;
                const size_t sx = pair_base + (size_t)(d * 2 + (ch & 1)) * KSX, sh = pair_base + 4 * KSX + (size_t)(d * 2 + (ch & 1)) * KSH;
                for (int n = 0; n < BR_NW; ++n) {
                    const int g = (n >> 1) & 3;
                    const int unit = ch * 16 + (n >> 3) * 2 + (n & 1);
                    const int wrow = g * H + unit;
                    const float scale = gate_scale(g);
                    bias[((size_t)d * BR_NCH + ch) * BR_NW + n] = scale * (bih[d][wrow] + bhh[d][wrow]);
                    for (int k = 0; k < K; ++k) put(n >> 5, sx + (k >> 6), n & 31, k & 63, scale * wih[d][(size_t)wrow * K + k]);
                    for (int k = 0; k < H; ++k) put(n >> 5, sh + (k >> 6), n & 31, k & 63, scale * whh[d][(size_t)wrow * H + k]);
                }
            }
        int rc;
        if ((rc = tc_alloc(m, (void**)&pk->w_img_dual, img.size()))) return rc;
        if ((rc = tc_alloc(m, (void**)&pk->bias_dual, bias.size() * sizeof(float)))) return rc;
        DSP_CUDA(cudaMemcpy(pk->w_img_dual, img.data(), img.size(), cudaMemcpyHostToDevice));
        DSP_CUDA(cudaMemcpy(pk->bias_dual, bias.data(), bias.size() * sizeof(float), cudaMemcpyHostToDevice));
    }
    const size_t per_rank = (size_t)NCH * KS;
    std::vector<uint8_t> img((size_t)2 * 2 * per_rank * HSLAB_BYTES, 0);
    std::vector<float> bias((size_t)2 * NCH * 128);
    for (int d = 0; d < 2; ++d)
        for (int ch = 0; ch < NCH; ++ch) {
            const size_t pair_base = (size_t)(ch >> 1) * 2 * KS;
            const size_t sx = pair_base + (size_t)(ch & 1) * KSX, sh = pair_base + 2 * KSX + (size_t)(ch & 1) * KSH;
            for (int n = 0; n < 128; ++n) {
                const int g = (n >> 1) & 3;
                const int unit = ch * 32 + (n >> 3) * 2 + (n & 1);
                const int wrow = g * H + unit;
                const float scale = gate_scale(g);
                const size_t rank_base = ((size_t)d * 2 + (n >> 6)) * per_rank;
                bias[((size_t)d * NCH + ch) * 128 + n] = scale * (bih[d][wrow] + bhh[d][wrow]);
                for (int k = 0; k < K; ++k)
                    put_half(img, rank_base, sx + (k >> 6), n, k & 63, scale * wih[d][(size_t)wrow * K + k]);
                for (int k = 0; k < H; ++k)
                    put_half(img, rank_base, sh + (k >> 6), n, k & 63, scale * whh[d][(size_t)wrow * H + k]);
            }
        }
    int rc;
    if ((rc = tc_alloc(m, (void**)&pk->w_img, img.size()))) return rc;
    if ((rc = tc_alloc(m, (void**)&pk->bias, bias.size() * sizeof(float)))) return rc;
    DSP_CUDA(cudaMemcpy(pk->w_img, img.data(), img.size(), cudaMemcpyHostToDevice));
    DSP_CUDA(cudaMemcpy(pk->bias, bias.data(), bias.size() * sizeof(float), cudaMemcpyHostToDevice));
    L.tc = pk;
    return DSP_OK;
}

int tc_pack_dense(Model* m, DenseF32& D, const float* w, const float* b) {
    TcState* s = (TcState*)m->tc_state;
    if (!(D.J == 128 || D.J == 256) || D.K != 2 * D.J) { D.tc = nullptr; return DSP_OK; }
    const int KS = D.K / 64, NCH = D.J / 128;
    TcDensePack* pk = new TcDensePack();
    s->dense_packs.push_back(pk);
    pk->KS = KS;
    const size_t per_rank = (size_t)NCH * KS;
    std::vector<uint8_t> img((size_t)2 * per_rank * HSLAB_BYTES, 0);
    for (int n = 0; n < D.J; ++n)
        for (int k = 0; k < D.K; ++k)
            put_half(img, (size_t)((n >> 6) & 1) * per_rank, (size_t)(n >> 7) * KS + (k >> 6), n & 127, k & 63, w[(size_t)n * D.K + k]);
    int rc;
    if ((rc = tc_alloc(m, (void**)&pk->w_img, img.size()))) return rc;
    if ((rc = tc_alloc(m, (void**)&pk->bias, sizeof(float) * D.J))) return rc;
    DSP_CUDA(cudaMemcpy(pk->w_img, img.data(), img.size(), cudaMemcpyHostToDevice));
    DSP_CUDA(cudaMemcpy(pk->bias, b, sizeof(float) * D.J, cudaMemcpyHostToDevice));
    D.tc = pk;
    return DSP_OK;
}

int tc_pack_head(Model* m, DenseF32& D, const float* w, const float* b) {
    TcState* s = (TcState*)m->tc_state;
    if (!(D.J == 256 && D.K == 512)) { s->tc_head = false; return DSP_OK; }
    const int KS = D.K / 64, NCH = D.J / 128;
    TcDensePack* pk = new TcDensePack();
    s->dense_packs.push_back(pk);
    s->head_pack = pk;
    pk->KS = KS;
    const size_t per_pass = (size_t)NCH * KS, per_rank = 3 * per_pass;
    std::vector<uint8_t> img((size_t)2 * per_rank * HSLAB_BYTES, 0);
    for (int n = 0; n < D.J; ++n)
        for (int k = 0; k < D.K; ++k) {
            const float wv = w[(size_t)n * D.K + k];
            const float hi = __half2float(__float2half_rn(wv));
            const size_t rank_base = (size_t)((n >> 6) & 1) * per_rank;
            const size_t slab = (size_t)(n >> 7) * KS + (k >> 6);
            put_half(img, rank_base, 0 * per_pass + slab, n & 127, k & 63, hi);
            put_half(img, rank_base, 1 * per_pass + slab, n & 127, k & 63, hi);
            put_half(img, rank_base, 2 * per_pass + slab, n & 127, k & 63, wv - hi);
        }
    int rc;
    if ((rc = tc_alloc(m, (void**)&pk->w_img, img.size()))) return rc;
    if ((rc = tc_alloc(m, (void**)&pk->bias, sizeof(float) * D.J))) return rc;
    DSP_CUDA(cudaMemcpy(pk->w_img, img.data(), img.size(), cudaMemcpyHostToDevice));
    DSP_CUDA(cudaMemcpy(pk->bias, b, sizeof(float) * D.J, cudaMemcpyHostToDevice));
    return DSP_OK;
}

int tc_forward_chunk(Model* m, const float* kmer, const float* means, const float* stds, const float* lens,
                     const float* signals, const float* const* h0, const float* const* c0,
                     const int64_t* sstride, uint64_t seed, uint64_t chunk_id, int64_t n,
                     float* logits, float* probs, int32_t* labels, cudaStream_t st) {
    TcState* s = (TcState*)m->tc_state;
    const dsp_config& c = m->cfg;
    const int T = c.seq_len, H = c.hidden_size;
    const int64_t tiles = ((n + TILE - 1) / TILE + 1) / 2 * 2;
    const bool seq = c.module != DSP_SIGNAL_BILSTM, sig = c.module != DSP_SEQ_BILSTM;
    {
        Span sp(m, 0, st);
        const int64_t total = tiles * TILE * T;
        cudaLaunchConfig_t cfg{};
        cfg.gridDim = dim3((unsigned)((total + 255) / 256));
        cfg.blockDim = dim3(256);
        cfg.stream = st;
        cudaLaunchAttribute attr[1];
        attr[0].id = cudaLaunchAttributeProgrammaticStreamSerialization;
        attr[0].val.programmaticStreamSerializationAllowed = 1;
        cfg.attrs = attr;
        cfg.numAttrs = s->pdl ? 1 : 0;
        DSP_CUDA(cudaLaunchKernelEx(&cfg, prep_images_kernel, kmer, means, stds, lens, signals, (const float*)m->embed,
                                    c.is_base ? c.embedding_size : 0, c.vocab_size, c.is_signallen, s->seq_split ? 1 : 0,
                                    c.signal_len, T, n, tiles * TILE, seq ? s->xseq_img : (uint8_t*)nullptr,
                                    sig ? s->xsig_img : (uint8_t*)nullptr));
        m->launches++;
    }
    auto run_stack = [&](std::vector<LstmLayer>& layers, const uint8_t* x0, int grp, int hid, bool is_comb) -> int {
        const uint8_t* x = x0;
        for (size_t l = 0; l < layers.size(); ++l) {
            TcLstmPack* pk = (TcLstmPack*)layers[l].tc;
            const bool final_layer = is_comb && l + 1 == layers.size();
            LayerParams p{};
            p.x_img = x; p.w_img = pk->w_img; p.bias = pk->bias;
            if (h0) {
                p.h0 = h0[grp] + (int64_t)l * 2 * sstride[grp]; p.c0 = c0[grp] + (int64_t)l * 2 * sstride[grp];
                p.state_dir_stride = sstride[grp];
            }
            p.seed = seed; p.rng_call = (uint32_t)chunk_id; p.rng_slot = (uint32_t)((grp * 8 + (int)l) * 2);
            p.site_base = (int64_t)chunk_id * m->cap;
            const bool head_tc = final_layer && s->tc_head;
            p.y_img = head_tc ? s->hfin_img : s->ybuf[l & 1]; p.hfinal = (final_layer && !head_tc) ? s->hfinal : nullptr;
            p.n = n; p.T = T; p.xk16 = pk->xk16; p.y_slabs = 2 * hid / 64; p.y_col_off = 0;
            p.write_y = final_layer ? (head_tc ? 2 : 0) : 1;
#ifdef DSP_MEAS_SKIP_Y
            if (p.write_y == 1 && hid == 256) { const char* e = getenv("DSP_B200_SKIP_Y_NOW"); if (e && atoi(e)) p.write_y = 0; }
#endif
            Span sp(m, is_comb ? 1 : 4, st);
            bool dual = pk->w_img_dual != nullptr;
            if (dual) {
                const int64_t sms = m->n_sm > 0 ? m->n_sm : 148;
                const double single_cost = (double)((2 * tiles + sms - 1) / sms);
                const double dual_cost = 1.8 * (double)((tiles + sms - 1) / sms);
                dual = dual_cost < single_cost;
                if (s->force_dual >= 0) dual = s->force_dual != 0;
            }
            if (dual) { p.w_img = pk->w_img_dual; p.bias = pk->bias_dual; }
            int rc = dual ? launch_branch<1>(m, p, tiles, st) : launch_lstm(m, pk->KSX, hid, p, tiles, st);
            if (rc) return rc;
            x = s->ybuf[l & 1];
        }
        return DSP_OK;
    };
    auto run_fc = [&](DenseF32& D, const uint8_t* x, int col_off) -> int {
        TcDensePack* pk = (TcDensePack*)D.tc;
        DSP_REQUIRE(pk != nullptr, DSP_ERR_INVALID, "tcgen05 path: dense layer %dx%d unsupported", D.J, D.K);
        LayerParams p{};
        p.x_img = x; p.w_img = pk->w_img; p.bias = pk->bias; p.y_img = s->comb_img; p.n = n; p.T = T;
        p.xk16 = pk->KS * 4; p.y_slabs = H / 64; p.y_col_off = col_off; p.write_y = 1;
        Span sp(m, 2, st);
        return launch_fc(m, pk->KS, D.J, p, tiles, st);
    };
    int rc;
    int comb_off = 0;
    bool fused = seq && sig && s->force_dual < 0 && m->lstm_seq.size() == 1 && m->lstm_signal.size() == 1 &&
                 m->nhid_seq == BR_H && m->nhid_signal == BR_H && H == 256;
    if (fused) {
        TcLstmPack* pk[2] = {(TcLstmPack*)m->lstm_seq[0].tc, (TcLstmPack*)m->lstm_signal[0].tc};
        TcDensePack* fk[2] = {(TcDensePack*)m->fc_seq.tc, (TcDensePack*)m->fc_signal.tc};
        fused = pk[0] && pk[1] && fk[0] && fk[1] && pk[0]->w_img_dual && pk[1]->w_img_dual && pk[0]->KSX == 1 && pk[1]->KSX == 1 &&
                fk[0]->KS == 4 && fk[1]->KS == 4;
        if (fused) {
            FusedBranchParams p{};
            const uint8_t* ximg[2] = {s->xseq_img, s->xsig_img};
            for (int b = 0; b < 2; ++b) {
                p.x_img[b] = ximg[b]; p.w_img[b] = pk[b]->w_img_dual; p.bias[b] = pk[b]->bias_dual;
                if (h0) { p.h0[b] = h0[b]; p.c0[b] = c0[b]; p.state_dir_stride[b] = sstride[b]; }
                p.rng_slot[b] = (uint32_t)((b * 8) * 2);
                p.xk16[b] = pk[b]->xk16;
                p.y_img[b] = s->ybuf[b];
                p.fcw_img[b] = fk[b]->w_img; p.fcb[b] = fk[b]->bias;
            }
            p.comb_img = s->comb_img; p.seed = seed; p.rng_call = (uint32_t)chunk_id; p.site_base = (int64_t)chunk_id * m->cap;
            p.n = n; p.T = T;
            Span sp(m, 4, st);
            if ((rc = launch_branch_fused(m, p, tiles, st))) return rc;
        }
    }
    if (fused) {
    } else if (seq) {
        if ((rc = run_stack(m->lstm_seq, s->xseq_img, 0, m->nhid_seq, false))) return rc;
        if ((rc = run_fc(m->fc_seq, s->ybuf[(m->lstm_seq.size() - 1) & 1], 0))) return rc;
        comb_off = m->nhid_seq;
    }
    if (!fused && sig) {
        if ((rc = run_stack(m->lstm_signal, s->xsig_img, 1, m->nhid_signal, false))) return rc;
        if ((rc = run_fc(m->fc_signal, s->ybuf[(m->lstm_signal.size() - 1) & 1], comb_off))) return rc;
    }
    if ((rc = run_stack(m->lstm_comb, s->comb_img, 2, H, true))) return rc;
    Span sp(m, 3, st);
    if (!s->tc_head) return f32_head_flat(m, s->hfinal, n, logits, probs, labels, st);
    TcDensePack* pk = s->head_pack;
    DSP_REQUIRE(pk != nullptr && pk->KS == 8 && m->fc1.J == 256, DSP_ERR_INVALID, "tcgen05 path: head shape unsupported");
    LayerParams p{};
    p.x_img = s->hfin_img; p.w_img = pk->w_img; p.bias = pk->bias; p.n = n; p.T = 3; p.xk16 = 32;
    p.w2t = m->fc2.wt; p.b2 = m->fc2.bias; p.logits = logits; p.probs = probs; p.labels = labels; p.num_classes = c.num_classes;
    return launch_layer<8, 0, MODE_HEAD, 256>(m, p, tiles, st);
}

}
```

deepsignal_plant_b200/csrc/tc_selftest.cu:

```cuda
#include "common.cuh"
#include "tc_prims.cuh"
#include <vector>
#include <cmath>
#include <cstdlib>

namespace dsp {
namespace {

using namespace tc;

__global__ void __launch_bounds__(128, 1)
selftest_kernel(const __half* __restrict__ a_slabs, const __half* __restrict__ a_rowmajor,
                const __half* __restrict__ b_slabs, float* __restrict__ d_out, int N, int KS, int a_in_tmem) {
    extern __shared__ __align__(1024) uint8_t smem_raw[];
    uint8_t* smem = (uint8_t*)(((uintptr_t)smem_raw + 1023) & ~(uintptr_t)1023);
    const int K = KS * SLAB_K;
    uint8_t* sA = smem;
    uint8_t* sB = sA + (size_t)KS * 128 * SLAB_ROW_BYTES;
    __shared__ __align__(8) uint64_t bars[2];
    __shared__ uint32_t tmem_base_s;
    const int tid = threadIdx.x, warp = tid >> 5;
    const uint32_t bar_load = smem_u32(&bars[0]), bar_mma = smem_u32(&bars[1]);
    if (tid == 0) {
        mbar_init(bar_load, 1);
        mbar_init(bar_mma, 1);
        mbar_fence_init();
    }
    if (warp == 0) tmem_alloc(smem_u32(&tmem_base_s), 512);
    tc_fence_before();
    __syncthreads();
    tc_fence_after();
    const uint32_t tmem = tmem_base_s;
    const uint32_t acc = tmem;
    const uint32_t a_t = tmem + 320;

    if (tid == 0) {
        const uint32_t a_bytes = a_in_tmem ? 0u : (uint32_t)KS * 128 * SLAB_ROW_BYTES;
        const uint32_t b_bytes = (uint32_t)KS * N * SLAB_ROW_BYTES;
        mbar_arrive_expect_tx(bar_load, a_bytes + b_bytes);
        if (!a_in_tmem) bulk_g2s(smem_u32(sA), a_slabs, a_bytes, bar_load);
        bulk_g2s(smem_u32(sB), b_slabs, b_bytes, bar_load);
    }
    if (a_in_tmem) {
        const __half* row = a_rowmajor + (size_t)tid * K;
        for (int k = 0; k < K; k += 16) {
            uint32_t v[8];
#pragma unroll
            for (int j = 0; j < 8; ++j) v[j] = pack_half2(__half2float(row[k + 2 * j]), __half2float(row[k + 2 * j + 1]));
            tmem_st8(a_t + ((uint32_t)(warp * 32) << 16) + (uint32_t)(k / 2), v);
        }
        tmem_st_wait();
    }
    tc_fence_before();
    __syncthreads();
    tc_fence_after();
    if (tid == 0) {
        mbar_wait(bar_load, 0);
        tc_fence_after();
        const uint32_t idesc = make_idesc_f16(128, N);
        for (int ks = 0; ks < KS; ++ks) {
            for (int k = 0; k < 4; ++k) {
                const uint64_t bd = make_smem_desc(smem_u32(sB + (size_t)ks * N * SLAB_ROW_BYTES) + k * 32);
                const uint32_t accum = (ks | k) ? 1u : 0u;
                if (a_in_tmem) {
                    mma_ts(acc, a_t + (uint32_t)((ks * SLAB_K + k * 16) / 2), bd, idesc, accum);
                } else {
                    const uint64_t ad = make_smem_desc(smem_u32(sA + (size_t)ks * 128 * SLAB_ROW_BYTES) + k * 32);
                    mma_ss(acc, ad, bd, idesc, accum);
                }
            }
        }
        mma_commit(bar_mma);
    }
    mbar_wait(bar_mma, 0);
    tc_fence_after();
    for (int c0 = 0; c0 < N; c0 += 32) {
        uint32_t v[32];
        tmem_ld32(acc + ((uint32_t)(warp * 32) << 16) + (uint32_t)c0, v);
        tmem_ld_wait();
#pragma unroll
        for (int j = 0; j < 32; ++j) d_out[(size_t)tid * N + c0 + j] = __uint_as_float(v[j]);
    }
    tc_fence_before();
    __syncthreads();
    if (warp == 0) tmem_dealloc(tmem, 512);
}

__global__ void __launch_bounds__(256, 1)
mma_rate_kernel(const uint8_t* __restrict__ src, int iters, int mode, unsigned long long* __restrict__ cycles_out) {
    extern __shared__ __align__(1024) uint8_t smem_raw[];
    uint8_t* smem = (uint8_t*)(((uintptr_t)smem_raw + 1023) & ~(uintptr_t)1023);
    uint8_t* sA = smem;
    uint8_t* sB = smem + 16384;
    uint8_t* sL = smem + 49152;
    __shared__ __align__(8) uint64_t bars[4];
    __shared__ uint32_t tmem_base_s;
    __shared__ volatile int stop_flag;
    const int tid = threadIdx.x, warp = tid >> 5;
    for (int i = tid; i < 49152 / 4; i += blockDim.x) reinterpret_cast<uint32_t*>(smem)[i] = 0;
    if (tid == 0) {
        for (int i = 0; i < 4; ++i) mbar_init(smem_u32(&bars[i]), 1);
        mbar_fence_init();
        stop_flag = 0;
    }
    if (warp == 0) tmem_alloc(smem_u32(&tmem_base_s), 512);
    fence_proxy_async_smem();
    tc_fence_before();
    __syncthreads();
    tc_fence_after();
    const uint32_t tmem = tmem_base_s;
    const int N = (mode & 64) ? 64 : (mode & 2) ? 256 : 128;
    const int chains = 1 << ((mode >> 4) & 3);
    const uint32_t idesc = make_idesc_f16(128, N);
    if (warp == 0) {
        const bool leader = elect_one();
        const uint32_t a_lo = smem_desc_lo(smem_u32(sA)), b_lo = smem_desc_lo(smem_u32(sB));
        const uint32_t d0 = tmem, d1 = tmem + (uint32_t)((chains > 1) ? N : 0);
        const long long t0 = clock64();
        if (mode & 1) {
            for (int it = 0; it < iters; ++it) {
                if (leader) {
#pragma unroll
                    for (int k = 0; k < 8; ++k)
                        mma_ts_lo<1>((k & 1) ? d1 : d0, tmem + 384 + (k & 3) * 8, b_lo + (k & 3) * 2, idesc);
                }
                __syncwarp();
            }
        } else {
            for (int it = 0; it < iters; ++it) {
                if (leader) {
#pragma unroll
                    for (int k = 0; k < 8; ++k)
                        mma_ss_lo<1>((k & 1) ? d1 : d0, a_lo + (k & 3) * 2, b_lo + (k & 3) * 2, idesc);
                }
                __syncwarp();
            }
        }
        if (leader) mma_commit(smem_u32(&bars[0]));
        __syncwarp();
        mbar_wait(smem_u32(&bars[0]), 0);
        const long long t1 = clock64();
        if (leader) { cycles_out[blockIdx.x] = (unsigned long long)(t1 - t0); stop_flag = 1; }
    } else if (warp == 1 && (mode & 4)) {
        if (tid == 32) {
            uint32_t ph[2] = {0, 0};
            int buf = 0;
            size_t off = (size_t)blockIdx.x * 65536;
            while (!stop_flag) {
                const uint32_t bar = smem_u32(&bars[1 + buf]);
                mbar_arrive_expect_tx(bar, 32768);
                bulk_g2s(smem_u32(sL + buf * 32768), src + (off & ((64u << 20) - 1)), 32768, bar);
                off += 32768;
                if (buf == 1) {
                    mbar_wait(smem_u32(&bars[1]), ph[0]); ph[0] ^= 1;
                    mbar_wait(smem_u32(&bars[2]), ph[1]); ph[1] ^= 1;
                }
                buf ^= 1;
            }
            if (buf == 1) { mbar_wait(smem_u32(&bars[1]), ph[0]); }
        }
    } else if (warp >= 4 && (mode & 8)) {
        uint32_t acc = 0;
        while (!stop_flag) {
            uint32_t v[32];
            tmem_ld32(tmem + ((uint32_t)((warp & 3) * 32) << 16) + 256, v);
            tmem_ld_wait();
            acc += v[0] + v[31];
        }
        if (acc == 0x12345678u) cycles_out[0] = 0;
    }
    tc_fence_before();
    __syncthreads();
    if (warp == 0) tmem_dealloc(tmem, 512);
}

__global__ void __launch_bounds__(512, 1)
pipe_probe_kernel(int iters, int mode, float seed, unsigned long long* __restrict__ cycles_out, float* __restrict__ sink) {
    float2 a[8];
    float e[8];
#pragma unroll
    for (int i = 0; i < 8; ++i) { a[i] = make_float2(seed + i, seed - i); e[i] = seed * 0.001f * (i + 1); }
    const float2 m = make_float2(0.999f, 1.001f), c = make_float2(1e-3f, -1e-3f);
    __syncthreads();
    const long long t0 = clock64();
    for (int it = 0; it < iters; ++it) {
#pragma unroll
        for (int i = 0; i < 8; ++i) {
            if (mode & 1) e[i] = ex2_approx(e[i]);
            if (mode & 8) e[i] = rcp_approx(e[i]);
            if (mode & 2) a[i] = fma2(a[i], m, c);
            if (mode & 4) { a[i].x = fmaf(a[i].x, m.x, c.x); a[i].y = fmaf(a[i].y, m.y, c.y); }
        }
    }
    const long long t1 = clock64();
    __syncthreads();
    float acc = 0.f;
#pragma unroll
    for (int i = 0; i < 8; ++i) acc += a[i].x + a[i].y + e[i];
    if (acc == 12345.678f) sink[0] = acc;
    if (threadIdx.x == 0) cycles_out[blockIdx.x] = (unsigned long long)(t1 - t0);
}

void to_slabs(const std::vector<__half>& m, int rows, int K, std::vector<__half>& out) {
    const int KS = K / SLAB_K;
    out.assign((size_t)rows * K, __float2half(0.f));
    for (int ks = 0; ks < KS; ++ks)
        for (int r = 0; r < rows; ++r)
            for (int c = 0; c < SLAB_K; ++c) {
                size_t off = (size_t)ks * rows * SLAB_ROW_BYTES + slab_offset_bytes(r, c);
                out[off / 2] = m[(size_t)r * K + ks * SLAB_K + c];
            }
}

}
}

using namespace dsp;

extern "C" int dsp_selftest(int device, int which, double* max_abs_err) {
    DSP_REQUIRE(max_abs_err, DSP_ERR_INVALID, "dsp_selftest: null output");
    *max_abs_err = -1.0;
    int ndev = 0;
    if (cudaGetDeviceCount(&ndev) != cudaSuccess || ndev == 0) {
        cudaGetLastError();
        set_error("dsp_selftest: no CUDA device available");
        return DSP_ERR_CUDA;
    }
    DSP_REQUIRE(device >= 0 && device < ndev, DSP_ERR_INVALID, "dsp_selftest: bad device");
    DSP_REQUIRE((which >= 0 && which <= 3) || (which >= 100 && which < 228) || (which >= 300 && which < 316), DSP_ERR_INVALID,
                "dsp_selftest: unknown test %d", which);
    DSP_CUDA(cudaSetDevice(device));
    if (which >= 300) {
        const int mode = which - 300, iters = 4000;
        int nsm = 0;
        DSP_CUDA(cudaDeviceGetAttribute(&nsm, cudaDevAttrMultiProcessorCount, device));
        unsigned long long* cyc; float* sink;
        DSP_CUDA(cudaMalloc(&cyc, sizeof(unsigned long long) * nsm));
        DSP_CUDA(cudaMalloc(&sink, sizeof(float)));
        for (int rep = 0; rep < 2; ++rep) {
            pipe_probe_kernel<<<nsm, 512>>>(iters, mode, 0.5f, cyc, sink);
            DSP_CUDA(cudaGetLastError());
            DSP_CUDA(cudaDeviceSynchronize());
        }
        std::vector<unsigned long long> h(nsm);
        DSP_CUDA(cudaMemcpy(h.data(), cyc, sizeof(unsigned long long) * nsm, cudaMemcpyDeviceToHost));
        cudaFree(cyc); cudaFree(sink);
        double sum = 0;
        for (auto v : h) sum += (double)v;
        *max_abs_err = sum / nsm / (double)iters;
        return DSP_OK;
    }
    if (which >= 100) {
        const int mode = which - 100, iters = 2000;
        int nsm = 0;
        DSP_CUDA(cudaDeviceGetAttribute(&nsm, cudaDevAttrMultiProcessorCount, device));
        uint8_t* src; unsigned long long* cyc;
        DSP_CUDA(cudaMalloc(&src, (size_t)64 << 20));
        DSP_CUDA(cudaMemset(src, 0, (size_t)64 << 20));
        DSP_CUDA(cudaMalloc(&cyc, sizeof(unsigned long long) * nsm));
        const size_t smem = 49152 + 65536 + 1024;
        DSP_CUDA(cudaFuncSetAttribute(mma_rate_kernel, cudaFuncAttributeMaxDynamicSharedMemorySize, (int)smem));
        for (int rep = 0; rep < 2; ++rep) {
            mma_rate_kernel<<<nsm, 256, smem>>>(src, iters, mode, cyc);
            DSP_CUDA(cudaGetLastError());
            DSP_CUDA(cudaDeviceSynchronize());
        }
        std::vector<unsigned long long> h(nsm);
        DSP_CUDA(cudaMemcpy(h.data(), cyc, sizeof(unsigned long long) * nsm, cudaMemcpyDeviceToHost));
        cudaFree(src); cudaFree(cyc);
        double sum = 0;
        for (auto v : h) sum += (double)v;
        *max_abs_err = sum / nsm / ((double)iters * 8);
        return DSP_OK;
    }
    const int N = (which == 1 || which == 3) ? 256 : 128;
    const int KS = which == 0 ? 1 : which == 1 ? 3 : which == 2 ? 2 : 4;
    const int K = KS * tc::SLAB_K;
    const int a_in_tmem = which >= 2;
    std::vector<__half> A((size_t)128 * K), B((size_t)N * K), As, Bs;
    srand(1234 + which);
    for (auto& v : A) v = __float2half((float)(rand() % 2001 - 1000) / 1000.f);
    for (auto& v : B) v = __float2half((float)(rand() % 2001 - 1000) / 1000.f);
    to_slabs(A, 128, K, As);
    to_slabs(B, N, K, Bs);
    __half *dA, *dAr, *dB; float* dD;
    DSP_CUDA(cudaMalloc(&dA, As.size() * 2));
    DSP_CUDA(cudaMalloc(&dAr, A.size() * 2));
    DSP_CUDA(cudaMalloc(&dB, Bs.size() * 2));
    DSP_CUDA(cudaMalloc(&dD, (size_t)128 * N * 4));
    DSP_CUDA(cudaMemcpy(dA, As.data(), As.size() * 2, cudaMemcpyHostToDevice));
    DSP_CUDA(cudaMemcpy(dAr, A.data(), A.size() * 2, cudaMemcpyHostToDevice));
    DSP_CUDA(cudaMemcpy(dB, Bs.data(), Bs.size() * 2, cudaMemcpyHostToDevice));
    DSP_CUDA(cudaMemset(dD, 0xff, (size_t)128 * N * 4));
    const size_t smem = (size_t)KS * (128 + N) * tc::SLAB_ROW_BYTES + 1024;
    DSP_CUDA(cudaFuncSetAttribute(selftest_kernel, cudaFuncAttributeMaxDynamicSharedMemorySize, (int)smem));
    selftest_kernel<<<1, 128, smem>>>(dA, dAr, dB, dD, N, KS, a_in_tmem);
    DSP_CUDA(cudaGetLastError());
    DSP_CUDA(cudaDeviceSynchronize());
    std::vector<float> D((size_t)128 * N);
    DSP_CUDA(cudaMemcpy(D.data(), dD, D.size() * 4, cudaMemcpyDeviceToHost));
    cudaFree(dA); cudaFree(dAr); cudaFree(dB); cudaFree(dD);
    double worst = 0.0;
    for (int m = 0; m < 128; ++m)
        for (int n = 0; n < N; ++n) {
            double ref = 0.0;
            for (int k = 0; k < K; ++k) ref += (double)__half2float(A[(size_t)m * K + k]) * (double)__half2float(B[(size_t)n * K + k]);
            double e = std::fabs(ref - (double)D[(size_t)m * N + n]);
            if (!(e <= worst)) worst = std::isnan(e) ? 1e30 : e;
        }
    *max_abs_err = worst;
    return DSP_OK;
}
```

Before: 9.581 million.

## Keep branch LSTM weights resident in shared memory and unify branch kernels

Replaces the per-timestep streamed weight ring in the dual-direction branch LSTM kernel with a layout where the full W_hh and packed W_ih (only the needed K16 groups) stay resident in shared memory. This removes the repeated global-to-shared weight reloads and the associated cluster barrier traffic every step. It also merges the separate and fused branch kernels into one templated kernel and adds a selftest for sub-slab B group addressing. The cost is higher shared memory use and a tighter limit on input width (xk16 up to 3).

```diff
diff --git a/deepsignal_plant_b200/csrc/kernels_tc.cu b/deepsignal_plant_b200/csrc/kernels_tc.cu
--- a/deepsignal_plant_b200/csrc/kernels_tc.cu
+++ b/deepsignal_plant_b200/csrc/kernels_tc.cu
@@ -612,298 +612,22 @@
 }
 
 constexpr int BR_H = 128, BR_NW = 64, BR_NCH = BR_H / 16, BR_KSH = BR_H / 64;
+constexpr int BR_NBIAS = 2 * BR_NCH * BR_NW;
 constexpr int QSLAB_BYTES = 32 * SLAB_ROW_BYTES;
-constexpr int BR_STG = 4, BR_NST = 6;
-
-template <int KSX>
-__global__ void __launch_bounds__(NTHREADS, 1)
-branch_kernel(const LayerParams p) {
-    constexpr int KS = KSX + BR_KSH;
-    constexpr int PAIR_UNITS = 4 * KSX + 4 * BR_KSH;
-    constexpr int W_STEP = (BR_NCH / 2) * PAIR_UNITS;
-    constexpr int NBIAS = 2 * BR_NCH * BR_NW;
-    constexpr uint32_t IDESC = make_idesc_f16(256, BR_NW);
-    static_assert(W_STEP % BR_STG == 0 && KS * 2 == PAIR_UNITS / 2, "stream layout");
-
-    extern __shared__ __align__(1024) uint8_t smem_raw[];
-    uint8_t* smem = (uint8_t*)(((uintptr_t)smem_raw + 1023) & ~(uintptr_t)1023);
-    uint8_t* s_x = smem;
-    uint8_t* s_w = smem + (size_t)2 * KSX * SLAB_BYTES;
-    float* s_bias = reinterpret_cast<float*>(s_w + (size_t)BR_NST * BR_STG * QSLAB_BYTES);
-    __shared__ __align__(8) uint64_t bars[2 * BR_NST + 4 * KSX + 10];
-    __shared__ uint32_t tmem_base_s;
-    const uint32_t b_wfull = smem_u32(&bars[0]), b_wempty = smem_u32(&bars[BR_NST]);
-    const uint32_t b_xfull = smem_u32(&bars[2 * BR_NST]), b_xempty = b_xfull + 8 * 2 * KSX;
-    const uint32_t b_accfull = b_xempty + 8 * 2 * KSX, b_accempty = b_accfull + 32;
-    const uint32_t b_hready = b_accempty + 32;
-
-    const int tid = threadIdx.x, warp = tid >> 5, lane = tid & 31;
-    const int tile = blockIdx.x;
-    const int T = p.T;
-    const uint32_t crank = cluster_ctarank();
-
-    if (tid == 0) {
-        const uint32_t both = crank == 0 ? 2u : 1u;
-        for (int i = 0; i < BR_NST; ++i) { mbar_init(b_wfull + 8 * i, both); mbar_init(b_wempty + 8 * i, 1); }
-        for (int i = 0; i < 2 * KSX; ++i) { mbar_init(b_xfull + 8 * i, both); mbar_init(b_xempty + 8 * i, 1); }
-        for (int i = 0; i < 4; ++i) { mbar_init(b_accfull + 8 * i, 1); mbar_init(b_accempty + 8 * i, EPI_WARPS); }
-        for (int i = 0; i < 2; ++i) mbar_init(b_hready + 8 * i, EPI_WARPS);
-        mbar_fence_init();
-    }
-    if (warp == 3) tmem_alloc_pair(smem_u32(&tmem_base_s), 512);
-    tc_fence_before();
-    __syncthreads();
-    cluster_sync_all();
-    tc_fence_after();
-    const uint32_t tmem = tmem_base_s;
-    griddep_launch_dependents();
-    auto t_acc = [&](int d, int e) -> uint32_t { return tmem + (uint32_t)(d * 128 + e * 64); };
-    auto t_h = [&](int d, int b) -> uint32_t { return tmem + 256u + (uint32_t)(d * 128 + b * 64); };
-
-    if (warp < 4) {
-        asm volatile("setmaxnreg.dec.sync.aligned.u32 32;");
-        if (warp == 0) {
-            if (elect_one()) {
-                const uint8_t* wsrc = p.w_img + (size_t)crank * W_STEP * QSLAB_BYTES;
-                uint32_t stage = 0, phase = 0;
-                for (int step = 0; step < T; ++step) {
-                    const uint8_t* src = wsrc;
-                    for (int s = 0; s < W_STEP; s += BR_STG) {
-                        mbar_wait(b_wempty + 8 * stage, phase ^ 1);
-                        mbar_arrive_expect_tx(b_wfull + 8 * stage, BR_STG * QSLAB_BYTES);
-                        bulk_g2s(smem_u32(s_w + (size_t)stage * BR_STG * QSLAB_BYTES), src, BR_STG * QSLAB_BYTES, b_wfull + 8 * stage);
-                        src += (size_t)BR_STG * QSLAB_BYTES;
-                        if (++stage == BR_NST) { stage = 0; phase ^= 1; }
-                    }
-                }
-            }
-        } else if (warp == 2) {
-            if (elect_one()) {
-                griddep_wait();
-                for (int step = 0; step < T; ++step)
-                    for (int d = 0; d < 2; ++d) {
-                        const int t = d ? (T - 1 - step) : step;
-                        const uint8_t* xsrc = p.x_img + ((size_t)tile * T + t) * KSX * SLAB_BYTES;
-                        for (int j = 0; j < KSX; ++j) {
-                            const uint32_t o = 8u * (uint32_t)(d * KSX + j);
-                            mbar_wait(b_xempty + o, (step & 1) ^ 1);
-                            mbar_arrive_expect_tx(b_xfull + o, SLAB_BYTES);
-                            bulk_g2s(smem_u32(s_x + (size_t)(d * KSX + j) * SLAB_BYTES), xsrc + (size_t)j * SLAB_BYTES, SLAB_BYTES, b_xfull + o);
-                        }
-                    }
-            }
-        } else if (warp == 1 && crank != 0) {
-            const uint32_t r_wfull = mapa_u32(b_wfull, 0), r_xfull = mapa_u32(b_xfull, 0);
-            uint32_t stage = 0, phase = 0;
-            for (int step = 0; step < T; ++step) {
-                for (int i = 0; i < 2 * KSX; ++i) {
-                    mbar_wait(b_xfull + 8 * i, step & 1);
-                    if (lane == 0) mbar_arrive_cluster(r_xfull + 8 * i);
-                }
-                for (int s = 0; s < W_STEP; s += BR_STG) {
-                    mbar_wait(b_wfull + 8 * stage, phase);
-                    if (lane == 0) mbar_arrive_cluster(r_wfull + 8 * stage);
-                    if (++stage == BR_NST) { stage = 0; phase ^= 1; }
-                }
-            }
-        } else if (warp == 1) {
-            const bool leader = elect_one();
-            const uint32_t a_lo0 = smem_desc_lo(smem_u32(s_x)), b_lo0 = smem_desc_lo(smem_u32(s_w));
-            const int xk16 = p.xk16;
-            uint32_t stage = 0, phase = 0, in_stage = 0;
-            auto w_acquire = [&]() -> uint32_t {
-                if (in_stage == 0) { mbar_wait_cluster(b_wfull + 8 * stage, phase); tc_fence_after(); }
-                return b_lo0 + (stage * BR_STG + in_stage) * (uint32_t)(QSLAB_BYTES >> 4);
-            };
-            auto w_release = [&]() {
-                if (++in_stage == BR_STG) {
-                    if (leader) mma2_commit(b_wempty + 8 * stage, PAIR_MASK);
-                    in_stage = 0;
-                    if (++stage == BR_NST) { stage = 0; phase ^= 1; }
-                }
-                __syncwarp();
-            };
-            for (int step = 0; step < T; ++step) {
-                for (int pr = 0; pr < BR_NCH / 2; ++pr) {
-                    const uint32_t use = (uint32_t)(step * (BR_NCH / 2) + pr);
-#pragma unroll
-                    for (int d = 0; d < 2; ++d)
-#pragma unroll
-                        for (int e = 0; e < 2; ++e) {
-                            mbar_wait_cluster(b_accempty + 8 * (d * 2 + e), (use & 1u) ^ 1u);
-                            tc_fence_after();
-#pragma unroll
-                            for (int j = 0; j < KSX; ++j) {
-                                const uint32_t xo = 8u * (uint32_t)(d * KSX + j);
-                                if (pr == 0 && e == 0) { mbar_wait_cluster(b_xfull + xo, step & 1); tc_fence_after(); }
-                                const uint32_t bl = w_acquire();
-                                if (leader) {
-                                    const uint32_t al = a_lo0 + (uint32_t)(d * KSX + j) * (SLAB_BYTES >> 4);
-                                    const int nk = (KSX * 4 == xk16) ? 4 : min(4, xk16 - 4 * j);
-#pragma unroll
-                                    for (int k = 0; k < 4; ++k) {
-                                        if (k < nk) {
-                                            if (j == 0 && k == 0) mma2_ss_lo<0>(t_acc(d, e), al, bl, IDESC);
-                                            else mma2_ss_lo<1>(t_acc(d, e), al + k * 2, bl + k * 2, IDESC);
-                                        }
-                                    }
-                                    if (pr == BR_NCH / 2 - 1 && e == 1) mma2_commit(b_xempty + xo, PAIR_MASK);
-                                }
-                                w_release();
-                            }
-                        }
-#pragma unroll
-                    for (int d = 0; d < 2; ++d) {
-                        if (pr == 0) { mbar_wait_cluster(b_hready + 8 * d, step & 1); tc_fence_after(); }
-                        const uint32_t a_t = t_h(d, step & 1);
-#pragma unroll
-                        for (int e = 0; e < 2; ++e) {
-#pragma unroll
-                            for (int j = 0; j < BR_KSH; ++j) {
-                                const uint32_t bl = w_acquire();
-                                if (leader) {
-#pragma unroll
-                                    for (int k = 0; k < 4; ++k)
-                                        mma2_ts_lo<1>(t_acc(d, e), a_t + (uint32_t)(j * 32 + k * 8), bl + k * 2, IDESC);
-                                }
-                                w_release();
-                            }
-                            if (leader) mma2_commit(b_accfull + 8 * (d * 2 + e), PAIR_MASK);
-                            __syncwarp();
-                        }
-                    }
-                }
-            }
-        }
-    } else {
-        asm volatile("setmaxnreg.inc.sync.aligned.u32 112;");
-        const int ew = warp - 4;
-        const int d = ew >> 3;
-        const int q = warp & 3;
-        const int half = (ew >> 2) & 1;
-        const int row = q * 32 + lane;
-        const int64_t site = (int64_t)tile * TILE + row;
-        const bool valid = site < p.n;
-        const uint32_t lane_addr = (uint32_t)(q * 32) << 16;
-        const uint32_t r_accempty = mapa_u32(b_accempty, 0) + 16u * (uint32_t)d, r_hready = mapa_u32(b_hready, 0) + 8u * (uint32_t)d;
-        const uint32_t b_myfull = b_accfull + 16u * (uint32_t)d;
-
-        for (int i = tid - 128; i < NBIAS; i += EPI_WARPS * 32) s_bias[i] = p.bias[i];
-        asm volatile("bar.sync 1, %0;" ::"n"(EPI_WARPS * 32) : "memory");
-
-        constexpr int UPT = 8;
-        float2 c2[BR_NCH][UPT / 2];
-        const bool draw = p.h0 == nullptr;
-        const uint64_t gs = (uint64_t)(p.site_base + site);
-        const uint32_t k0 = (uint32_t)p.seed, k1 = (uint32_t)(p.seed >> 32);
-        const uint32_t slot0 = (p.rng_slot + (uint32_t)d) << 16;
-        if (draw) {
-#pragma unroll 1
-            for (int i = 0; i < BR_NCH * (UPT / 4); ++i) {
-                const int unit = (i >> 1) * 16 + half * UPT + (i & 1) * 4;
-                const float4 hq = philox_normal4((uint32_t)gs, (uint32_t)(gs >> 32), slot0 | (uint32_t)(unit >> 2), p.rng_call, k0, k1);
-                tmem_st2(t_h(d, 0) + lane_addr + (uint32_t)(unit >> 1), pack_half2(hq.x, hq.y), pack_half2(hq.z, hq.w));
-            }
-            tmem_st_wait();
-        } else {
-            const float* h0 = p.h0 + (size_t)d * p.state_dir_stride + (size_t)site * BR_H;
-            const float* c0 = p.c0 + (size_t)d * p.state_dir_stride + (size_t)site * BR_H;
-#pragma unroll
-            for (int ch = 0; ch < BR_NCH; ++ch) {
-                const int u0 = ch * 16 + half * UPT;
-                float4 cv0 = make_float4(0.f, 0.f, 0.f, 0.f), cv1 = cv0, hq0 = cv0, hq1 = cv0;
-                if (valid) {
-                    cv0 = *reinterpret_cast<const float4*>(c0 + u0); cv1 = *reinterpret_cast<const float4*>(c0 + u0 + 4);
-                    hq0 = *reinterpret_cast<const float4*>(h0 + u0); hq1 = *reinterpret_cast<const float4*>(h0 + u0 + 4);
-                }
-                c2[ch][0] = make_float2(cv0.x, cv0.y); c2[ch][1] = make_float2(cv0.z, cv0.w);
-                c2[ch][2] = make_float2(cv1.x, cv1.y); c2[ch][3] = make_float2(cv1.z, cv1.w);
-                tmem_st4(t_h(d, 0) + lane_addr + (uint32_t)(u0 >> 1), pack_half2(hq0.x, hq0.y), pack_half2(hq0.z, hq0.w),
-                         pack_half2(hq1.x, hq1.y), pack_half2(hq1.z, hq1.w));
-            }
-            tmem_st_wait();
-        }
-        tc_fence_before();
-        __syncwarp();
-        if (lane == 0) mbar_arrive_cluster(r_hready);
-        if (draw) {
-            const uint32_t t_park = t_h(d, 1) + lane_addr;
-#pragma unroll 1
-            for (int i = 0; i < BR_NCH * (UPT / 4); ++i) {
-                const int unit = (i >> 1) * 16 + half * UPT + (i & 1) * 4;
-                const float4 cv = philox_normal4((uint32_t)gs, (uint32_t)(gs >> 32), slot0 | (uint32_t)(unit >> 2) | 0x8000u, p.rng_call, k0, k1);
-                tmem_st2(t_park + (uint32_t)(unit >> 1), pack_half2(cv.x, cv.y), pack_half2(cv.z, cv.w));
-            }
-            tmem_st_wait();
-#pragma unroll
-            for (int ch = 0; ch < BR_NCH; ++ch) {
-                uint32_t v[4];
-                tmem_ld4(t_park + (uint32_t)((ch * 16 + half * UPT) >> 1), v);
-                tmem_ld_wait();
-#pragma unroll
-                for (int j = 0; j < UPT / 2; ++j) {
-                    const __half2 hh = *reinterpret_cast<const __half2*>(&v[j]);
-                    c2[ch][j] = make_float2(__low2float(hh), __high2float(hh));
-                }
-            }
-        }
-        const uint32_t s_bias_u32 = smem_u32(s_bias) + (uint32_t)((d * BR_NCH * BR_NW + half * 32) * 4);
-        for (int step = 0; step < T; ++step) {
-            const int t = d ? (T - 1 - step) : step;
-            uint8_t* ybase = p.y_img + ((size_t)tile * T + t) * p.y_slabs * SLAB_BYTES + row * SLAB_ROW_BYTES;
-            const uint32_t t_hnext = t_h(d, (step + 1) & 1) + lane_addr;
-#pragma unroll
-            for (int ch = 0; ch < BR_NCH; ++ch) {
-                const int e = ch & 1;
-                const uint32_t use = (uint32_t)(step * (BR_NCH / 2) + (ch >> 1));
-                mbar_wait(b_myfull + 8 * e, use & 1u);
-                tc_fence_after();
-                const int u0 = ch * 16 + half * UPT;
-                float2 h2[UPT / 2];
-#pragma unroll
-                for (int part = 0; part < 2; ++part) {
-                    uint32_t v[16];
-                    tmem_ld16(t_acc(d, e) + lane_addr + (uint32_t)(half * 32 + part * 16), v);
-                    float4 bq[4];
-#pragma unroll
-                    for (int i = 0; i < 4; ++i) bq[i] = lds128(s_bias_u32 + (uint32_t)((ch * BR_NW + part * 16 + i * 4) * 4));
-                    tmem_ld_wait();
-                    if (part == 1) {
-                        tc_fence_before();
-                        __syncwarp();
-                        if (lane == 0) mbar_arrive_cluster(r_accempty + 8 * e);
-                    }
-#pragma unroll
-                    for (int qq = 0; qq < 2; ++qq) {
-                        const float4 b0 = bq[2 * qq], b1 = bq[2 * qq + 1];
-                        const float2 ai = add2(make_float2(__uint_as_float(v[qq * 8 + 0]), __uint_as_float(v[qq * 8 + 1])), make_float2(b0.x, b0.y));
-                        const float2 af = add2(make_float2(__uint_as_float(v[qq * 8 + 2]), __uint_as_float(v[qq * 8 + 3])), make_float2(b0.z, b0.w));
-                        const float2 ag = add2(make_float2(__uint_as_float(v[qq * 8 + 4]), __uint_as_float(v[qq * 8 + 5])), make_float2(b1.x, b1.y));
-                        const float2 ao = add2(make_float2(__uint_as_float(v[qq * 8 + 6]), __uint_as_float(v[qq * 8 + 7])), make_float2(b1.z, b1.w));
-                        lstm_cell2<DSP_POLY_MASK_BRANCH>(ai, af, ag, ao, c2[ch][part * 2 + qq], h2[part * 2 + qq]);
-                    }
-                }
-                uint32_t pk[UPT / 2];
-#pragma unroll
-                for (int j = 0; j < UPT / 2; ++j) pk[j] = pack_half2(h2[j].x, h2[j].y);
-                tmem_st4(t_hnext + (uint32_t)(u0 >> 1), pk[0], pk[1], pk[2], pk[3]);
-                const int col = d * BR_H + u0;
-                uint8_t* yslab = ybase + (size_t)(col >> 6) * SLAB_BYTES;
-                *reinterpret_cast<uint4*>(yslab + ((((col & 63) >> 3) ^ (row & 7)) << 4)) = make_uint4(pk[0], pk[1], pk[2], pk[3]);
-            }
-            tmem_st_wait();
-            tc_fence_before();
-            __syncwarp();
-            if (lane == 0) mbar_arrive_cluster(r_hready);
-        }
-    }
-    tc_fence_before();
-    __syncthreads();
-    cluster_sync_all();
-    if (warp == 3) tmem_dealloc_pair(tmem, 512);
-}
-
-struct FusedBranchParams {
+constexpr int BR_WHH_BYTES = 2 * BR_NCH * BR_KSH * QSLAB_BYTES;
+constexpr int BR_MAX_XK16 = 3;
+__host__ __device__ constexpr int br_wih_bytes(int xk16) { return 2 * BR_NCH * xk16 / 4 * QSLAB_BYTES; }
+constexpr int BR_X_OFF = 0;
+constexpr int BR_W_OFF = 2 * SLAB_BYTES;
+constexpr int BR_BIAS_OFF = BR_W_OFF + BR_WHH_BYTES + br_wih_bytes(BR_MAX_XK16);
+constexpr int BR_FC_KS = 4;
+constexpr int BR_NA = 8;
+constexpr int BR_A_OFF = BR_FC_KS * HSLAB_BYTES;
+constexpr size_t BR_SMEM = (size_t)BR_BIAS_OFF + (BR_NBIAS + 128) * sizeof(float) + 1024;
+static_assert(BR_A_OFF + BR_NA * SLAB_BYTES <= BR_BIAS_OFF, "tail ring fits in the space of x_t + weights");
+static_assert(BR_SMEM <= 227 * 1024, "shared memory of one CTA");
+
+struct BranchParams {
     const uint8_t* x_img[2];
     const uint8_t* w_img[2];
     const float* bias[2];
@@ -923,55 +647,50 @@
     int T;
 };
 
+template <bool FC>
 __global__ void __launch_bounds__(NTHREADS, 1)
-branch_fused_kernel(const FusedBranchParams p) {
-    constexpr int KSX = 1;
-    constexpr int KS = KSX + BR_KSH;
-    constexpr int PAIR_UNITS = 4 * KSX + 4 * BR_KSH;
-    constexpr int W_STEP = (BR_NCH / 2) * PAIR_UNITS;
-    constexpr int NBIAS = 2 * BR_NCH * BR_NW;
+branch_kernel(const BranchParams p) {
     constexpr uint32_t IDESC = make_idesc_f16(256, BR_NW);
     constexpr uint32_t IDESC_FC = make_idesc_f16(256, 128);
-    constexpr int FC_KS = 4;
-    static_assert(W_STEP % BR_STG == 0 && KS * 2 == PAIR_UNITS / 2, "stream layout");
-    static_assert(2 * KSX * SLAB_BYTES + BR_NST * BR_STG * QSLAB_BYTES == 2 * FC_KS * SLAB_BYTES, "tail A buffers alias x + ring exactly");
+    constexpr uint32_t QS = QSLAB_BYTES >> 4, SS = SLAB_BYTES >> 4;
 
     extern __shared__ __align__(1024) uint8_t smem_raw[];
     uint8_t* smem = (uint8_t*)(((uintptr_t)smem_raw + 1023) & ~(uintptr_t)1023);
-    uint8_t* s_x = smem;
-    uint8_t* s_w = smem + (size_t)2 * KSX * SLAB_BYTES;
-    uint8_t* s_a = smem;
-    uint8_t* s_wfc = smem + (size_t)2 * FC_KS * SLAB_BYTES;
-    float* s_bias = reinterpret_cast<float*>(s_wfc + (size_t)FC_KS * HSLAB_BYTES);
-    float* s_fcb = s_bias + NBIAS;
-    __shared__ __align__(8) uint64_t bars[2 * BR_NST + 4 * KSX + 10 + 10];
+    uint8_t* s_x = smem + BR_X_OFF;
+    uint8_t* s_w = smem + BR_W_OFF;
+    uint8_t* s_wfc = smem + BR_X_OFF;
+    uint8_t* s_a = smem + BR_A_OFF;
+    float* s_bias = reinterpret_cast<float*>(smem + BR_BIAS_OFF);
+    float* s_fcb = s_bias + BR_NBIAS;
+    __shared__ __align__(8) uint64_t bars[1 + 4 + 8 + 2 + 2 + 2 * BR_NA + 8];
     __shared__ uint32_t tmem_base_s;
-    const uint32_t b_wfull = smem_u32(&bars[0]), b_wempty = smem_u32(&bars[BR_NST]);
-    const uint32_t b_xfull = smem_u32(&bars[2 * BR_NST]), b_xempty = b_xfull + 8 * 2 * KSX;
-    const uint32_t b_accfull = b_xempty + 8 * 2 * KSX, b_accempty = b_accfull + 32;
+    const uint32_t b_wfull = smem_u32(&bars[0]);
+    const uint32_t b_xfull = b_wfull + 8, b_xempty = b_xfull + 16;
+    const uint32_t b_accfull = b_xempty + 16, b_accempty = b_accfull + 32;
     const uint32_t b_hready = b_accempty + 32;
     const uint32_t b_tail = b_hready + 16;
     const uint32_t b_wfc = b_tail + 8;
-    const uint32_t b_afull = b_wfc + 8, b_aempty = b_afull + 16;
-    const uint32_t b_faccfull = b_aempty + 16, b_faccempty = b_faccfull + 16;
+    const uint32_t b_afull = b_wfc + 8, b_aempty = b_afull + 8 * BR_NA;
+    const uint32_t b_faccfull = b_aempty + 8 * BR_NA, b_faccempty = b_faccfull + 32;
 
     const int tid = threadIdx.x, warp = tid >> 5, lane = tid & 31;
-    const int br = (int)((blockIdx.x >> 1) & 1u);
-    const int tile = (int)(((blockIdx.x >> 2) << 1) | (blockIdx.x & 1u));
+    const int br = FC ? (int)((blockIdx.x >> 1) & 1u) : 0;
+    const int tile = FC ? (int)(((blockIdx.x >> 2) << 1) | (blockIdx.x & 1u)) : (int)blockIdx.x;
     const int T = p.T;
+    const int xk16 = p.xk16[br];
     const uint32_t crank = cluster_ctarank();
 
     if (tid == 0) {
         const uint32_t both = crank == 0 ? 2u : 1u;
-        for (int i = 0; i < BR_NST; ++i) { mbar_init(b_wfull + 8 * i, both); mbar_init(b_wempty + 8 * i, 1); }
-        for (int i = 0; i < 2 * KSX; ++i) { mbar_init(b_xfull + 8 * i, both); mbar_init(b_xempty + 8 * i, 1); }
+        mbar_init(b_wfull, both);
+        for (int i = 0; i < 2; ++i) { mbar_init(b_xfull + 8 * i, both); mbar_init(b_xempty + 8 * i, 1); }
         for (int i = 0; i < 4; ++i) { mbar_init(b_accfull + 8 * i, 1); mbar_init(b_accempty + 8 * i, EPI_WARPS); }
         for (int i = 0; i < 2; ++i) mbar_init(b_hready + 8 * i, EPI_WARPS);
-        mbar_init(b_tail, EPI_WARPS);
-        mbar_init(b_wfc, both);
-        for (int i = 0; i < 2; ++i) {
-            mbar_init(b_afull + 8 * i, both); mbar_init(b_aempty + 8 * i, 1);
-            mbar_init(b_faccfull + 8 * i, 1); mbar_init(b_faccempty + 8 * i, 2 * EPI_WARPS);
+        if (FC) {
+            mbar_init(b_tail, EPI_WARPS);
+            mbar_init(b_wfc, both);
+            for (int i = 0; i < BR_NA; ++i) { mbar_init(b_afull + 8 * i, both); mbar_init(b_aempty + 8 * i, 1); }
+            for (int i = 0; i < 4; ++i) { mbar_init(b_faccfull + 8 * i, 1); mbar_init(b_faccempty + 8 * i, 2 * EPI_WARPS); }
         }
         mbar_fence_init();
     }
@@ -989,159 +708,129 @@
 
     if (warp < 4) {
         asm volatile("setmaxnreg.dec.sync.aligned.u32 32;");
-        if (warp == 0) {
+        if (warp == 0 || warp == 2) {
             if (elect_one()) {
-                mbar_arrive_expect_tx(b_wfc, FC_KS * HSLAB_BYTES);
-                bulk_g2s(smem_u32(s_wfc), p.fcw_img[br] + (size_t)crank * FC_KS * HSLAB_BYTES, FC_KS * HSLAB_BYTES, b_wfc);
-                const uint8_t* wsrc = p.w_img[br] + (size_t)crank * W_STEP * QSLAB_BYTES;
-                uint32_t stage = 0, phase = 0;
+                const int d = warp >> 1;
+                if (d == 0) {
+                    const uint32_t wbytes = (uint32_t)(BR_WHH_BYTES + br_wih_bytes(xk16));
+                    const uint8_t* wsrc = p.w_img[br] + (size_t)crank * wbytes;
+                    mbar_arrive_expect_tx(b_wfull, wbytes);
+                    for (uint32_t o = 0; o < wbytes; o += SLAB_BYTES)
+                        bulk_g2s(smem_u32(s_w + o), wsrc + o, SLAB_BYTES, b_wfull);
+                }
+                griddep_wait();
+                const uint32_t xf = b_xfull + 8 * d, xe = b_xempty + 8 * d;
                 for (int step = 0; step < T; ++step) {
-                    const uint8_t* src = wsrc;
-                    for (int s = 0; s < W_STEP; s += BR_STG) {
-                        mbar_wait(b_wempty + 8 * stage, phase ^ 1);
-                        mbar_arrive_expect_tx(b_wfull + 8 * stage, BR_STG * QSLAB_BYTES);
-                        bulk_g2s(smem_u32(s_w + (size_t)stage * BR_STG * QSLAB_BYTES), src, BR_STG * QSLAB_BYTES, b_wfull + 8 * stage);
-                        src += (size_t)BR_STG * QSLAB_BYTES;
-                        if (++stage == BR_NST) { stage = 0; phase ^= 1; }
-                    }
-                }
-            }
-        } else if (warp == 2) {
-            if (elect_one()) {
-                griddep_wait();
-                for (int step = 0; step < T; ++step)
-                    for (int d = 0; d < 2; ++d) {
-                        const int t = d ? (T - 1 - step) : step;
-                        const uint8_t* xsrc = x_img + ((size_t)tile * T + t) * KSX * SLAB_BYTES;
-                        for (int j = 0; j < KSX; ++j) {
-                            const uint32_t o = 8u * (uint32_t)(d * KSX + j);
-                            mbar_wait(b_xempty + o, (step & 1) ^ 1);
-                            mbar_arrive_expect_tx(b_xfull + o, SLAB_BYTES);
-                            bulk_g2s(smem_u32(s_x + (size_t)(d * KSX + j) * SLAB_BYTES), xsrc + (size_t)j * SLAB_BYTES, SLAB_BYTES, b_xfull + o);
+                    const int t = d ? (T - 1 - step) : step;
+                    mbar_wait(xe, (step & 1) ^ 1);
+                    mbar_arrive_expect_tx(xf, SLAB_BYTES);
+                    bulk_g2s(smem_u32(s_x + (size_t)d * SLAB_BYTES), x_img + ((size_t)tile * T + t) * SLAB_BYTES, SLAB_BYTES, xf);
+                }
+                if (FC && d == 0) {
+                    mbar_wait(b_tail, 0);
+                    mbar_arrive_expect_tx(b_wfc, BR_FC_KS * HSLAB_BYTES);
+                    bulk_g2s(smem_u32(s_wfc), p.fcw_img[br] + (size_t)crank * BR_FC_KS * HSLAB_BYTES, BR_FC_KS * HSLAB_BYTES, b_wfc);
+                    const uint8_t* ysrc = y_img + (size_t)tile * T * BR_FC_KS * SLAB_BYTES;
+                    for (int u = 0; u < T * BR_FC_KS; ++u) {
+                        const int slot = u % BR_NA;
+                        mbar_wait(b_aempty + 8 * slot, ((u / BR_NA) & 1) ^ 1);
+                        mbar_arrive_expect_tx(b_afull + 8 * slot, SLAB_BYTES);
+                        bulk_g2s(smem_u32(s_a + (size_t)slot * SLAB_BYTES), ysrc + (size_t)u * SLAB_BYTES, SLAB_BYTES, b_afull + 8 * slot);
+                    }
+                }
+            }
+        } else if (crank != 0) {
+            const int d = warp >> 1;
+            if (d == 0) {
+                mbar_wait(b_wfull, 0);
+                if (lane == 0) mbar_arrive_cluster(mapa_u32(b_wfull, 0));
+            }
+            const uint32_t xf = b_xfull + 8 * d, r_xfull = mapa_u32(xf, 0);
+            for (int step = 0; step < T; ++step) {
+                mbar_wait(xf, step & 1);
+                if (lane == 0) mbar_arrive_cluster(r_xfull);
+            }
+            if (FC && d == 0) {
+                mbar_wait(b_wfc, 0);
+                if (lane == 0) mbar_arrive_cluster(mapa_u32(b_wfc, 0));
+                const uint32_t r_afull = mapa_u32(b_afull, 0);
+                for (int u = 0; u < T * BR_FC_KS; ++u) {
+                    const int slot = u % BR_NA;
+                    mbar_wait(b_afull + 8 * slot, (u / BR_NA) & 1);
+                    if (lane == 0) mbar_arrive_cluster(r_afull + 8 * slot);
+                }
+            }
+        } else {
+            const int d = warp >> 1;
+            const bool leader = elect_one();
+            const uint32_t x_lo = smem_desc_lo(smem_u32(s_x)) + (uint32_t)d * SS;
+            const uint32_t hh_lo = smem_desc_lo(smem_u32(s_w)) + (uint32_t)(d * BR_NCH * BR_KSH) * QS;
+            const uint32_t ih_lo = smem_desc_lo(smem_u32(s_w + BR_WHH_BYTES));
+            const uint32_t xf = b_xfull + 8 * d, xe = b_xempty + 8 * d;
+            mbar_wait_cluster(b_wfull, 0);
+            tc_fence_after();
+            for (int use = 0; use < T * (BR_NCH / 2); ++use) {
+                const int step = use / (BR_NCH / 2), pr = use % (BR_NCH / 2);
+                const uint32_t a_t = t_h(d, step & 1);
+#pragma unroll
+                for (int e = 0; e < 2; ++e) {
+                    mbar_wait_cluster(b_accempty + 8 * (d * 2 + e), (use & 1u) ^ 1u);
+                    tc_fence_after();
+                    if (pr == 0 && e == 0) { mbar_wait_cluster(xf, step & 1); tc_fence_after(); }
+                    if (leader) {
+                        const int g0 = (d * BR_NCH + 2 * pr + e) * xk16;
+                        for (int k = 0; k < xk16; ++k) {
+                            const int g = g0 + k;
+                            const uint32_t bl = ih_lo + (uint32_t)(g >> 2) * QS + (uint32_t)(g & 3) * 2;
+                            if (k == 0) mma2_ss_lo<0>(t_acc(d, e), x_lo, bl, IDESC);
+                            else mma2_ss_lo<1>(t_acc(d, e), x_lo + k * 2, bl, IDESC);
                         }
-                    }
-                mbar_wait(b_tail, 0);
+                        if (pr == BR_NCH / 2 - 1 && e == 1) mma2_commit(xe, PAIR_MASK);
+                    }
+                    __syncwarp();
+                }
+                if (pr == 0) { mbar_wait_cluster(b_hready + 8 * d, step & 1); tc_fence_after(); }
+#pragma unroll
+                for (int e = 0; e < 2; ++e) {
+                    if (leader) {
+                        const uint32_t bl = hh_lo + (uint32_t)((2 * pr + e) * BR_KSH) * QS;
+#pragma unroll
+                        for (int j = 0; j < BR_KSH; ++j)
+#pragma unroll
+                            for (int k = 0; k < 4; ++k)
+                                mma2_ts_lo<1>(t_acc(d, e), a_t + (uint32_t)(j * 32 + k * 8), bl + (uint32_t)j * QS + k * 2, IDESC);
+                        mma2_commit(b_accfull + 8 * (d * 2 + e), PAIR_MASK);
+                    }
+                    __syncwarp();
+                }
+            }
+            if (FC && d == 0) {
+                const uint32_t fa_lo0 = smem_desc_lo(smem_u32(s_a)), fb_lo0 = smem_desc_lo(smem_u32(s_wfc));
+                mbar_wait_cluster(b_wfc, 0);
+                tc_fence_after();
                 for (int t = 0; t < T; ++t) {
-                    const uint32_t buf = (uint32_t)t & 1u;
-                    mbar_wait(b_aempty + 8 * buf, ((uint32_t)(t >> 1) & 1u) ^ 1u);
-                    mbar_arrive_expect_tx(b_afull + 8 * buf, FC_KS * SLAB_BYTES);
-                    bulk_g2s(smem_u32(s_a + (size_t)buf * FC_KS * SLAB_BYTES), y_img + ((size_t)tile * T + t) * FC_KS * SLAB_BYTES,
-                             FC_KS * SLAB_BYTES, b_afull + 8 * buf);
-                }
-            }
-        } else if (warp == 1 && crank != 0) {
-            const uint32_t r_wfull = mapa_u32(b_wfull, 0), r_xfull = mapa_u32(b_xfull, 0);
-            uint32_t stage = 0, phase = 0;
-            for (int step = 0; step < T; ++step) {
-                for (int i = 0; i < 2 * KSX; ++i) {
-                    mbar_wait(b_xfull + 8 * i, step & 1);
-                    if (lane == 0) mbar_arrive_cluster(r_xfull + 8 * i);
-                }
-                for (int s = 0; s < W_STEP; s += BR_STG) {
-                    mbar_wait(b_wfull + 8 * stage, phase);
-                    if (lane == 0) mbar_arrive_cluster(r_wfull + 8 * stage);
-                    if (++stage == BR_NST) { stage = 0; phase ^= 1; }
-                }
-            }
-            const uint32_t r_wfc = mapa_u32(b_wfc, 0), r_afull = mapa_u32(b_afull, 0);
-            mbar_wait(b_wfc, 0);
-            if (lane == 0) mbar_arrive_cluster(r_wfc);
-            for (int t = 0; t < T; ++t) {
-                const uint32_t buf = (uint32_t)t & 1u;
-                mbar_wait(b_afull + 8 * buf, (uint32_t)(t >> 1) & 1u);
-                if (lane == 0) mbar_arrive_cluster(r_afull + 8 * buf);
-            }
-        } else if (warp == 1) {
-            const bool leader = elect_one();
-            const uint32_t a_lo0 = smem_desc_lo(smem_u32(s_x)), b_lo0 = smem_desc_lo(smem_u32(s_w));
-            const int xk16 = p.xk16[br];
-            uint32_t stage = 0, phase = 0, in_stage = 0;
-            auto w_acquire = [&]() -> uint32_t {
-                if (in_stage == 0) { mbar_wait_cluster(b_wfull + 8 * stage, phase); tc_fence_after(); }
-                return b_lo0 + (stage * BR_STG + in_stage) * (uint32_t)(QSLAB_BYTES >> 4);
-            };
-            auto w_release = [&]() {
-                if (++in_stage == BR_STG) {
-                    if (leader) mma2_commit(b_wempty + 8 * stage, PAIR_MASK);
-                    in_stage = 0;
-                    if (++stage == BR_NST) { stage = 0; phase ^= 1; }
-                }
-                __syncwarp();
-            };
-            for (int step = 0; step < T; ++step) {
-                for (int pr = 0; pr < BR_NCH / 2; ++pr) {
-                    const uint32_t use = (uint32_t)(step * (BR_NCH / 2) + pr);
-#pragma unroll
-                    for (int d = 0; d < 2; ++d)
-#pragma unroll
-                        for (int e = 0; e < 2; ++e) {
-                            mbar_wait_cluster(b_accempty + 8 * (d * 2 + e), (use & 1u) ^ 1u);
-                            tc_fence_after();
-#pragma unroll
-                            for (int j = 0; j < KSX; ++j) {
-                                const uint32_t xo = 8u * (uint32_t)(d * KSX + j);
-                                if (pr == 0 && e == 0) { mbar_wait_cluster(b_xfull + xo, step & 1); tc_fence_after(); }
-                                const uint32_t bl = w_acquire();
-                                if (leader) {
-                                    const uint32_t al = a_lo0 + (uint32_t)(d * KSX + j) * (SLAB_BYTES >> 4);
-                                    const int nk = (KSX * 4 == xk16) ? 4 : min(4, xk16 - 4 * j);
-#pragma unroll
-                                    for (int k = 0; k < 4; ++k) {
-                                        if (k < nk) {
-                                            if (j == 0 && k == 0) mma2_ss_lo<0>(t_acc(d, e), al, bl, IDESC);
-                                            else mma2_ss_lo<1>(t_acc(d, e), al + k * 2, bl + k * 2, IDESC);
-                                        }
-                                    }
-                                    if (pr == BR_NCH / 2 - 1 && e == 1) mma2_commit(b_xempty + xo, PAIR_MASK);
-                                }
-                                w_release();
+                    const uint32_t buf = (uint32_t)t & 3u, use = (uint32_t)(t >> 2);
+                    mbar_wait_cluster(b_faccempty + 8 * buf, (use & 1u) ^ 1u);
+                    tc_fence_after();
+#pragma unroll
+                    for (int j = 0; j < BR_FC_KS; ++j) {
+                        const int u = t * BR_FC_KS + j, slot = u % BR_NA;
+                        mbar_wait_cluster(b_afull + 8 * slot, (u / BR_NA) & 1);
+                        tc_fence_after();
+                        if (leader) {
+                            const uint32_t al = fa_lo0 + (uint32_t)slot * SS, bl = fb_lo0 + (uint32_t)j * (HSLAB_BYTES >> 4);
+#pragma unroll
+                            for (int k = 0; k < 4; ++k) {
+                                if (j == 0 && k == 0) mma2_ss_lo<0>(tmem + buf * 128u, al, bl, IDESC_FC);
+                                else mma2_ss_lo<1>(tmem + buf * 128u, al + k * 2, bl + k * 2, IDESC_FC);
                             }
+                            mma2_commit(b_aempty + 8 * slot, PAIR_MASK);
                         }
-#pragma unroll
-                    for (int d = 0; d < 2; ++d) {
-                        if (pr == 0) { mbar_wait_cluster(b_hready + 8 * d, step & 1); tc_fence_after(); }
-                        const uint32_t a_t = t_h(d, step & 1);
-#pragma unroll
-                        for (int e = 0; e < 2; ++e) {
-#pragma unroll
-                            for (int j = 0; j < BR_KSH; ++j) {
-                                const uint32_t bl = w_acquire();
-                                if (leader) {
-#pragma unroll
-                                    for (int k = 0; k < 4; ++k)
-                                        mma2_ts_lo<1>(t_acc(d, e), a_t + (uint32_t)(j * 32 + k * 8), bl + k * 2, IDESC);
-                                }
-                                w_release();
-                            }
-                            if (leader) mma2_commit(b_accfull + 8 * (d * 2 + e), PAIR_MASK);
-                            __syncwarp();
-                        }
-                    }
-                }
-            }
-            const uint32_t fa_lo0 = smem_desc_lo(smem_u32(s_a)), fb_lo0 = smem_desc_lo(smem_u32(s_wfc));
-            mbar_wait_cluster(b_wfc, 0);
-            tc_fence_after();
-            for (int t = 0; t < T; ++t) {
-                const uint32_t buf = (uint32_t)t & 1u, use = (uint32_t)(t >> 1);
-                mbar_wait_cluster(b_faccempty + 8 * buf, (use & 1u) ^ 1u);
-                mbar_wait_cluster(b_afull + 8 * buf, use & 1u);
-                tc_fence_after();
-                if (leader) {
-#pragma unroll
-                    for (int j = 0; j < FC_KS; ++j) {
-                        const uint32_t al = fa_lo0 + (buf * FC_KS + (uint32_t)j) * (SLAB_BYTES >> 4);
-                        const uint32_t bl = fb_lo0 + (uint32_t)j * (HSLAB_BYTES >> 4);
-#pragma unroll
-                        for (int k = 0; k < 4; ++k) {
-                            if (j == 0 && k == 0) mma2_ss_lo<0>(tmem + buf * 128u, al, bl, IDESC_FC);
-                            else mma2_ss_lo<1>(tmem + buf * 128u, al + k * 2, bl + k * 2, IDESC_FC);
-                        }
-                    }
-                    mma2_commit(b_aempty + 8 * buf, PAIR_MASK);
-                    mma2_commit(b_faccfull + 8 * buf, PAIR_MASK);
-                }
-                __syncwarp();
+                        __syncwarp();
+                    }
+                    if (leader) mma2_commit(b_faccfull + 8 * buf, PAIR_MASK);
+                    __syncwarp();
+                }
             }
         }
     } else {
@@ -1157,8 +846,8 @@
         const uint32_t r_accempty = mapa_u32(b_accempty, 0) + 16u * (uint32_t)d, r_hready = mapa_u32(b_hready, 0) + 8u * (uint32_t)d;
         const uint32_t b_myfull = b_accfull + 16u * (uint32_t)d;
 
-        for (int i = tid - 128; i < NBIAS; i += EPI_WARPS * 32) s_bias[i] = p.bias[br][i];
-        for (int i = tid - 128; i < 128; i += EPI_WARPS * 32) s_fcb[i] = p.fcb[br][i];
+        for (int i = tid - 128; i < BR_NBIAS; i += EPI_WARPS * 32) s_bias[i] = p.bias[br][i];
+        if (FC) for (int i = tid - 128; i < 128; i += EPI_WARPS * 32) s_fcb[i] = p.fcb[br][i];
         asm volatile("bar.sync 1, %0;" ::"n"(EPI_WARPS * 32) : "memory");
 
         constexpr int UPT = 8;
@@ -1220,7 +909,7 @@
         const uint32_t s_bias_u32 = smem_u32(s_bias) + (uint32_t)((d * BR_NCH * BR_NW + half * 32) * 4);
         for (int step = 0; step < T; ++step) {
             const int t = d ? (T - 1 - step) : step;
-            uint8_t* ybase = y_img + ((size_t)tile * T + t) * FC_KS * SLAB_BYTES + row * SLAB_ROW_BYTES;
+            uint8_t* ybase = y_img + ((size_t)tile * T + t) * BR_FC_KS * SLAB_BYTES + row * SLAB_ROW_BYTES;
             const uint32_t t_hnext = t_h(d, (step + 1) & 1) + lane_addr;
 #pragma unroll
             for (int ch = 0; ch < BR_NCH; ++ch) {
@@ -1266,16 +955,16 @@
             __syncwarp();
             if (lane == 0) mbar_arrive_cluster(r_hready);
         }
-        asm volatile("fence.proxy.async.global;" ::: "memory");
-        __syncwarp();
-        if (lane == 0) mbar_arrive(b_tail);
-        {
+        if constexpr (FC) {
+            asm volatile("fence.proxy.async.global;" ::: "memory");
+            __syncwarp();
+            if (lane == 0) mbar_arrive(b_tail);
             const int sl = ew >> 2;
             const uint32_t r_faccempty = mapa_u32(b_faccempty, 0);
             const int col0 = br * 128 + sl * 32;
             const float* bs = s_fcb + sl * 32;
             for (int t = 0; t < T; ++t) {
-                const uint32_t buf = (uint32_t)t & 1u, use = (uint32_t)(t >> 1);
+                const uint32_t buf = (uint32_t)t & 3u, use = (uint32_t)(t >> 2);
                 mbar_wait(b_faccfull + 8 * buf, use & 1u);
                 tc_fence_after();
                 uint32_t v[32];
@@ -1284,7 +973,7 @@
                 tc_fence_before();
                 __syncwarp();
                 if (lane == 0) mbar_arrive_cluster(r_faccempty + 8 * buf);
-                uint8_t* yslab = p.comb_img + (((size_t)tile * T + t) * FC_KS + (size_t)(col0 >> 6)) * SLAB_BYTES + row * SLAB_ROW_BYTES;
+                uint8_t* yslab = p.comb_img + (((size_t)tile * T + t) * BR_FC_KS + (size_t)(col0 >> 6)) * SLAB_BYTES + row * SLAB_ROW_BYTES;
 #pragma unroll
                 for (int c8 = 0; c8 < 4; ++c8) {
                     uint32_t o[4];
@@ -1386,6 +1075,7 @@
     uint8_t* w_img = nullptr;
     float* bias = nullptr;
     int KSX = 0, xk16 = 0;
+
     uint8_t* w_img_dual = nullptr;
     float* bias_dual = nullptr;
 };
@@ -1452,36 +1142,14 @@
     return DSP_OK;
 }
 
-template <int KSX>
-int launch_branch(Model* m, const LayerParams& p, int64_t tiles, cudaStream_t st) {
-    const size_t smem = (size_t)2 * KSX * SLAB_BYTES + (size_t)BR_NST * BR_STG * QSLAB_BYTES + (size_t)2 * BR_NCH * BR_NW * sizeof(float) + 1024;
-    auto kern = branch_kernel<KSX>;
-    DSP_CUDA(cudaFuncSetAttribute(kern, cudaFuncAttributeMaxDynamicSharedMemorySize, (int)smem));
+template <bool FC>
+int launch_branch(Model* m, const BranchParams& p, int64_t tiles, cudaStream_t st) {
+    auto kern = branch_kernel<FC>;
+    DSP_CUDA(cudaFuncSetAttribute(kern, cudaFuncAttributeMaxDynamicSharedMemorySize, (int)BR_SMEM));
     cudaLaunchConfig_t cfg{};
-    cfg.gridDim = dim3((unsigned)((tiles + 1) / 2 * 2), 1);
+    cfg.gridDim = dim3((unsigned)((FC ? 2 : 1) * ((tiles + 1) / 2 * 2)), 1);
     cfg.blockDim = dim3(NTHREADS);
-    cfg.dynamicSmemBytes = smem;
-    cfg.stream = st;
-    cudaLaunchAttribute attr[2];
-    attr[0].id = cudaLaunchAttributeClusterDimension;
-    attr[0].val.clusterDim.x = 2; attr[0].val.clusterDim.y = 1; attr[0].val.clusterDim.z = 1;
-    attr[1].id = cudaLaunchAttributeProgrammaticStreamSerialization;
-    attr[1].val.programmaticStreamSerializationAllowed = 1;
-    cfg.attrs = attr;
-    cfg.numAttrs = ((TcState*)m->tc_state)->pdl ? 2 : 1;
-    DSP_CUDA(cudaLaunchKernelEx(&cfg, kern, p));
-    m->launches++;
-    return DSP_OK;
-}
-
-int launch_branch_fused(Model* m, const FusedBranchParams& p, int64_t tiles, cudaStream_t st) {
-    const size_t smem = (size_t)2 * 4 * SLAB_BYTES + (size_t)4 * HSLAB_BYTES + (size_t)(2 * BR_NCH * BR_NW + 128) * sizeof(float) + 1024;
-    auto kern = branch_fused_kernel;
-    DSP_CUDA(cudaFuncSetAttribute(kern, cudaFuncAttributeMaxDynamicSharedMemorySize, (int)smem));
-    cudaLaunchConfig_t cfg{};
-    cfg.gridDim = dim3((unsigned)(2 * ((tiles + 1) / 2 * 2)), 1);
-    cfg.blockDim = dim3(NTHREADS);
-    cfg.dynamicSmemBytes = smem;
+    cfg.dynamicSmemBytes = BR_SMEM;
     cfg.stream = st;
     cudaLaunchAttribute attr[2];
     attr[0].id = cudaLaunchAttributeClusterDimension;
@@ -1604,26 +1272,29 @@
     pk->xk16 = (K + 15) / 16;
     const float* wih[2] = {wih0, wih1}; const float* whh[2] = {whh0, whh1};
     const float* bih[2] = {bih0, bih1}; const float* bhh[2] = {bhh0, bhh1};
-    if (H == BR_H && KSX == 1) {
-        const int pair_units = 4 * KSX + 4 * KSH;
-        const size_t per_rank = (size_t)(BR_NCH / 2) * pair_units;
-        std::vector<uint8_t> img((size_t)2 * per_rank * QSLAB_BYTES, 0);
+    if (H == BR_H && KSX == 1 && pk->xk16 <= BR_MAX_XK16) {
+        const int xk16 = pk->xk16;
+        const size_t per_rank = (size_t)BR_WHH_BYTES + br_wih_bytes(xk16);
+        std::vector<uint8_t> img((size_t)2 * per_rank, 0);
         std::vector<float> bias((size_t)2 * BR_NCH * BR_NW);
-        auto put = [&](int rank, size_t unit, int row, int k, float v) {
+        auto put = [&](int rank, size_t qslab, int row, int k, float v) {
             __half h = __float2half_rn(v);
-            memcpy(&img[((size_t)rank * per_rank + unit) * QSLAB_BYTES + slab_offset_bytes((uint32_t)row, (uint32_t)k)], &h, 2);
+            memcpy(&img[(size_t)rank * per_rank + qslab * QSLAB_BYTES + slab_offset_bytes((uint32_t)row, (uint32_t)k)], &h, 2);
         };
         for (int d = 0; d < 2; ++d)
             for (int ch = 0; ch < BR_NCH; ++ch) {
-                const size_t pair_base = (size_t)(ch >> 1) * pair_units;
-                const size_t sx = pair_base + (size_t)(d * 2 + (ch & 1)) * KSX, sh = pair_base + 4 * KSX + (size_t)(d * 2 + (ch & 1)) * KSH;
+                const size_t sh = (size_t)(d * BR_NCH + ch) * KSH;
+                const int gx = (d * BR_NCH + ch) * xk16;
                 for (int n = 0; n < BR_NW; ++n) {
                     const int g = (n >> 1) & 3;
                     const int unit = ch * 16 + (n >> 3) * 2 + (n & 1);
                     const int wrow = g * H + unit;
                     const float scale = gate_scale(g);
                     bias[((size_t)d * BR_NCH + ch) * BR_NW + n] = scale * (bih[d][wrow] + bhh[d][wrow]);
-                    for (int k = 0; k < K; ++k) put(n >> 5, sx + (k >> 6), n & 31, k & 63, scale * wih[d][(size_t)wrow * K + k]);
+                    for (int k = 0; k < K; ++k) {
+                        const int gk = gx + (k >> 4);
+                        put(n >> 5, BR_WHH_BYTES / QSLAB_BYTES + (gk >> 2), n & 31, (gk & 3) * 16 + (k & 15), scale * wih[d][(size_t)wrow * K + k]);
+                    }
                     for (int k = 0; k < H; ++k) put(n >> 5, sh + (k >> 6), n & 31, k & 63, scale * whh[d][(size_t)wrow * H + k]);
                 }
             }
@@ -1767,8 +1438,17 @@
                 dual = dual_cost < single_cost;
                 if (s->force_dual >= 0) dual = s->force_dual != 0;
             }
-            if (dual) { p.w_img = pk->w_img_dual; p.bias = pk->bias_dual; }
-            int rc = dual ? launch_branch<1>(m, p, tiles, st) : launch_lstm(m, pk->KSX, hid, p, tiles, st);
+            int rc;
+            if (dual) {
+                BranchParams bp{};
+                bp.x_img[0] = x; bp.w_img[0] = pk->w_img_dual; bp.bias[0] = pk->bias_dual;
+                bp.h0[0] = p.h0; bp.c0[0] = p.c0; bp.state_dir_stride[0] = p.state_dir_stride; bp.rng_slot[0] = p.rng_slot;
+                bp.xk16[0] = pk->xk16; bp.y_img[0] = p.y_img;
+                bp.seed = seed; bp.rng_call = p.rng_call; bp.site_base = p.site_base; bp.n = n; bp.T = T;
+                rc = launch_branch<false>(m, bp, tiles, st);
+            } else {
+                rc = launch_lstm(m, pk->KSX, hid, p, tiles, st);
+            }
             if (rc) return rc;
             x = s->ybuf[l & 1];
         }
@@ -1793,7 +1473,7 @@
         fused = pk[0] && pk[1] && fk[0] && fk[1] && pk[0]->w_img_dual && pk[1]->w_img_dual && pk[0]->KSX == 1 && pk[1]->KSX == 1 &&
                 fk[0]->KS == 4 && fk[1]->KS == 4;
         if (fused) {
-            FusedBranchParams p{};
+            BranchParams p{};
             const uint8_t* ximg[2] = {s->xseq_img, s->xsig_img};
             for (int b = 0; b < 2; ++b) {
                 p.x_img[b] = ximg[b]; p.w_img[b] = pk[b]->w_img_dual; p.bias[b] = pk[b]->bias_dual;
@@ -1806,7 +1486,7 @@
             p.comb_img = s->comb_img; p.seed = seed; p.rng_call = (uint32_t)chunk_id; p.site_base = (int64_t)chunk_id * m->cap;
             p.n = n; p.T = T;
             Span sp(m, 4, st);
-            if ((rc = launch_branch_fused(m, p, tiles, st))) return rc;
+            if ((rc = launch_branch<true>(m, p, tiles, st))) return rc;
         }
     }
     if (fused) {
diff --git a/deepsignal_plant_b200/csrc/tc_selftest.cu b/deepsignal_plant_b200/csrc/tc_selftest.cu
--- a/deepsignal_plant_b200/csrc/tc_selftest.cu
+++ b/deepsignal_plant_b200/csrc/tc_selftest.cu
@@ -11,7 +11,7 @@
 
 __global__ void __launch_bounds__(128, 1)
 selftest_kernel(const __half* __restrict__ a_slabs, const __half* __restrict__ a_rowmajor,
-                const __half* __restrict__ b_slabs, float* __restrict__ d_out, int N, int KS, int a_in_tmem) {
+                const __half* __restrict__ b_slabs, float* __restrict__ d_out, int N, int KS, int a_in_tmem, int b_group) {
     extern __shared__ __align__(1024) uint8_t smem_raw[];
     uint8_t* smem = (uint8_t*)(((uintptr_t)smem_raw + 1023) & ~(uintptr_t)1023);
     const int K = KS * SLAB_K;
@@ -58,7 +58,8 @@
         mbar_wait(bar_load, 0);
         tc_fence_after();
         const uint32_t idesc = make_idesc_f16(128, N);
-        for (int ks = 0; ks < KS; ++ks) {
+        if (b_group >= 0) mma_ss(acc, make_smem_desc(smem_u32(sA)), make_smem_desc(smem_u32(sB) + b_group * 32), idesc, 0u);
+        for (int ks = 0; ks < KS && b_group < 0; ++ks) {
             for (int k = 0; k < 4; ++k) {
                 const uint64_t bd = make_smem_desc(smem_u32(sB + (size_t)ks * N * SLAB_ROW_BYTES) + k * 32);
                 const uint32_t accum = (ks | k) ? 1u : 0u;
@@ -227,7 +228,7 @@
         return DSP_ERR_CUDA;
     }
     DSP_REQUIRE(device >= 0 && device < ndev, DSP_ERR_INVALID, "dsp_selftest: bad device");
-    DSP_REQUIRE((which >= 0 && which <= 3) || (which >= 100 && which < 228) || (which >= 300 && which < 316), DSP_ERR_INVALID,
+    DSP_REQUIRE((which >= 0 && which <= 4) || (which >= 100 && which < 228) || (which >= 300 && which < 316), DSP_ERR_INVALID,
                 "dsp_selftest: unknown test %d", which);
     DSP_CUDA(cudaSetDevice(device));
     if (which >= 300) {
@@ -274,9 +275,10 @@
         return DSP_OK;
     }
     const int N = (which == 1 || which == 3) ? 256 : 128;
-    const int KS = which == 0 ? 1 : which == 1 ? 3 : which == 2 ? 2 : 4;
+    const int KS = (which == 0 || which == 4) ? 1 : which == 1 ? 3 : which == 2 ? 2 : 4;
     const int K = KS * tc::SLAB_K;
-    const int a_in_tmem = which >= 2;
+    const int a_in_tmem = which == 2 || which == 3;
+    const int b_group = which == 4 ? 3 : -1;
     std::vector<__half> A((size_t)128 * K), B((size_t)N * K), As, Bs;
     srand(1234 + which);
     for (auto& v : A) v = __float2half((float)(rand() % 2001 - 1000) / 1000.f);
@@ -294,7 +296,7 @@
     DSP_CUDA(cudaMemset(dD, 0xff, (size_t)128 * N * 4));
     const size_t smem = (size_t)KS * (128 + N) * tc::SLAB_ROW_BYTES + 1024;
     DSP_CUDA(cudaFuncSetAttribute(selftest_kernel, cudaFuncAttributeMaxDynamicSharedMemorySize, (int)smem));
-    selftest_kernel<<<1, 128, smem>>>(dA, dAr, dB, dD, N, KS, a_in_tmem);
+    selftest_kernel<<<1, 128, smem>>>(dA, dAr, dB, dD, N, KS, a_in_tmem, b_group);
     DSP_CUDA(cudaGetLastError());
     DSP_CUDA(cudaDeviceSynchronize());
     std::vector<float> D((size_t)128 * N);
@@ -304,7 +306,12 @@
     for (int m = 0; m < 128; ++m)
         for (int n = 0; n < N; ++n) {
             double ref = 0.0;
-            for (int k = 0; k < K; ++k) ref += (double)__half2float(A[(size_t)m * K + k]) * (double)__half2float(B[(size_t)n * K + k]);
+            if (b_group >= 0) {
+                for (int k = 0; k < 16; ++k)
+                    ref += (double)__half2float(A[(size_t)m * K + k]) * (double)__half2float(B[(size_t)n * K + b_group * 16 + k]);
+            } else {
+                for (int k = 0; k < K; ++k) ref += (double)__half2float(A[(size_t)m * K + k]) * (double)__half2float(B[(size_t)n * K + k]);
+            }
             double e = std::fabs(ref - (double)D[(size_t)m * N + n]);
             if (!(e <= worst)) worst = std::isnan(e) ? 1e30 : e;
         }
```

Result: no change. 9.674 million (median of 6 runs) (+1.0%).
